# flanglet/kanzi

Measured on AMD Instinct MI355X. Metric: encode+decode MB/s, 4 MiB-block synthetic stream, BWT+RANK+ZRLT & ANS0 (level-5 core chain), bit-exact .knz, higher is better.
Workload: dtype u8; 1 GPU; configs[2]: BWT+RANK+ZRLT & ANS0, 2048 x 4194304 B blocks per GPU per step (64 distinct synthetic blocks per GPU, SURVEY 8d generator standing in for silesia.tar, tiled), blocks round-robin over ranks; block_size=4194304, parallelism=blocks%1, round_trip_ok=True

## Files before the change

kanzi_amd/csrc/kz_api.hip:

```cpp
#include <dirent.h>
#include "kz_device.h"
#include "kz_internal.h"
#include <stdlib.h>
#include <algorithm>
#include <atomic>
#include <memory>
#include <thread>
#include <chrono>
#include <sched.h>

typedef uint32_t u32;
typedef uint8_t u8;
typedef unsigned long long u64;

extern "C" int32_t kz_abi_version(void) { return KZ_ABI_VERSION; }

extern "C" kz_ctx* kz_ctx_create(int32_t deviceId) {
  int ndev = 0;
  if (hipGetDeviceCount(&ndev) != hipSuccess || ndev <= 0) return nullptr;
  if (deviceId < 0 || deviceId >= ndev) return nullptr;
  if (hipSetDevice(deviceId) != hipSuccess) return nullptr;
  kz_ctx* ctx = new kz_ctx();
  ctx->device = deviceId;
  { int cus = 0; if (hipDeviceGetAttribute(&cus, hipDeviceAttributeMultiprocessorCount, deviceId) == hipSuccess && cus > 0) ctx->numCUs = cus; }
  if (hipStreamCreateWithFlags(&ctx->stream, hipStreamNonBlocking) != hipSuccess) { delete ctx; return nullptr; }
  if (hipHostMalloc((void**)&ctx->hpin, 1 << 20, hipHostMallocDefault) != hipSuccess) { hipStreamDestroy(ctx->stream); delete ctx; return nullptr; }
  ctx->hpinInts = (1 << 20) / 4;
  kz_switches_read(ctx->sw);
  {
    const int hw = (int)std::thread::hardware_concurrency();
    ctx->blockingWaits = ctx->sw.blockingWaits >= 0 ? ctx->sw.blockingWaits : ((hw > 0 && kz_usable_cpus() < hw) ? 1 : 0);
  }
  return ctx;
}
void kz_switches_read(kz_switches& s) {
  s = kz_switches();
  auto num = [](const char* name, int unset) { const char* e = getenv(name); return e ? atoi(e) : unset; };
  auto flag = [](const char* name) { return getenv(name) != nullptr ? 1 : 0; };
  auto digit = [](const char* name, int lo, int hi, int unset) { const char* e = getenv(name); return (e && e[0] >= '0' + lo && e[0] <= '0' + hi) ? e[0] - '0' : unset; };
  { const char* e = getenv("KZ_BLOCKING_WAITS"); s.blockingWaits = e ? (atoi(e) ? 1 : 0) : -1; }
  s.textGpu = digit("KZ_TEXT_GPU", 0, 3, -1);
  s.textGpuMin = num("KZ_TEXT_GPU_MIN", 512);
  s.textFwdGpu = digit("KZ_TEXT_FWD_GPU", 0, 1, -1);
  s.textFwdGpuMin = num("KZ_TEXT_FWD_GPU_MIN", 256);
  s.utfGpu = digit("KZ_UTF_GPU", 0, 0, 1);
  s.utfFwdGpu = digit("KZ_UTF_FWD_GPU", 0, 1, -1);
  s.textGpuTrace = flag("KZ_TEXT_GPU_TRACE");
  s.fuseMinBlocks = num("KZ_FUSE_MIN_BLOCKS", 32);
  s.overlapClasses = num("KZ_OVERLAP_CLASSES", 3);
  { const char* e = getenv("KZ_WIDE_QUEUES"); s.wideQueues = e ? (atoi(e) ? 1 : 0) : -1; }
  s.noSFirst = flag("KZ_NO_SFIRST");
  s.traceSched = flag("KZ_TRACE_SCHED");
  s.tracePipe = flag("KZ_TRACE_PIPE");
  s.hostChunk = num("KZ_HOST_CHUNK", 0);
  { const int v = num("KZ_HOST_CHUNK_DEC", 512); s.hostChunkDec = v < 8 ? 8 : v; }
  { const char* e = getenv("KZ_HOST_INV_STAGED"); s.hostInvStaged = e ? atoi(e) : -1; }
  s.streamChunk = num("KZ_STREAM_CHUNK", 0);
  s.streamSerial = flag("KZ_STREAM_SERIAL");
  s.bwtTrie = num("KZ_BWT_TRIE", -1); s.bwtTrieWin = num("KZ_BWT_TRIEWIN", -1); s.bwtBuckets = num("KZ_BWT_BUCKETS", -1);
  s.bwtDmax = num("KZ_BWT_DMAX", -1); s.bwtRetire = num("KZ_BWT_RETIRE", -1); s.bwtLazyRank = num("KZ_BWT_LAZYRANK", -1);
  s.bwtTrace = flag("KZ_BWT_TRACE");
  s.bwtTestTrieOverflow = digit("KZ_BWT_TEST_TRIE_OVERFLOW", 0, 9, -1);
  { const char* f = getenv("KZ_FPAQ_FORCE"); s.fpaqForce = f ? ((f[0] == 'w' || f[0] == 'W' || f[0] == '1') ? 1 : ((f[0] == 'l' || f[0] == 'L' || f[0] == '2') ? 2 : 0)) : 0; }
  s.sbrtForm = num("KZ_SBRT_FORM", -1);
}
extern "C" void kz_ctx_reload_switches(kz_ctx* ctx) {
  if (!ctx) return;
  kz_switches_read(ctx->sw);
  if (ctx->sw.blockingWaits >= 0) ctx->blockingWaits = ctx->sw.blockingWaits;
}
extern "C" void kz_ctx_destroy(kz_ctx* ctx) {
  if (!ctx) return;
  if (ctx->worker.joinable()) {
    { std::lock_guard<std::mutex> g(ctx->qmu); ctx->stopWorker = true; }
    ctx->qcv.notify_all();
    ctx->worker.join();
  }
  hipSetDevice(ctx->device);
  if (ctx->arena) hipFree(ctx->arena);
  for (int i = 0; i < 5; i++) { if (ctx->side[i]) hipStreamDestroy(ctx->side[i]); if (ctx->evJoin[i]) hipEventDestroy(ctx->evJoin[i]); }
  if (ctx->hpin) hipHostFree(ctx->hpin);
  for (int i = 0; i < 2; i++) {
    if (ctx->pinIn[i].p) hipHostFree(ctx->pinIn[i].p);
    if (ctx->pinOut[i].p) hipHostFree(ctx->pinOut[i].p);
    if (ctx->hsIn[i].p) hipHostFree(ctx->hsIn[i].p);
    if (ctx->hsOut[i].p) hipHostFree(ctx->hsOut[i].p);
    if (ctx->tfOut[i].p) hipHostFree(ctx->tfOut[i].p);
    if (ctx->hiAux[i].p) hipFree(ctx->hiAux[i].p);
    if (ctx->hiStream[i]) hipStreamDestroy(ctx->hiStream[i]);
    if (ctx->devIn[i].p) hipFree(ctx->devIn[i].p);
    if (ctx->devOut[i].p) hipFree(ctx->devOut[i].p);
  }
  if (ctx->tfIn.p) hipHostFree(ctx->tfIn.p);
  if (ctx->tfCopy) hipStreamDestroy(ctx->tfCopy);
  if (ctx->evBlock) hipEventDestroy(ctx->evBlock);
  if (ctx->copyUp) hipStreamDestroy(ctx->copyUp);
  if (ctx->copyDown) hipStreamDestroy(ctx->copyDown);
  if (ctx->stream) hipStreamDestroy(ctx->stream);
  delete ctx;
}
extern "C" int32_t kz_ctx_set_checksum(kz_ctx* ctx, int32_t bits) {
  if (!ctx || (bits != 0 && bits != 32 && bits != 64)) return -KZ_ERR_INVALID_PARAM;
  ctx->checksum = bits == 32 ? 1 : (bits == 64 ? 2 : 0);
  return 0;
}
extern "C" int32_t kz_ctx_set_skip_blocks(kz_ctx* ctx, int32_t on) {
  if (!ctx) return -KZ_ERR_INVALID_PARAM;
  ctx->skipBlocks = on ? 1 : 0;
  return 0;
}
extern "C" int32_t kz_ctx_set_data_type(kz_ctx* ctx, int32_t dataType) {
  if (!ctx || dataType < KZ_DT_UNDEFINED || dataType > KZ_DT_UTF8) return -KZ_ERR_INVALID_PARAM;
  ctx->dataType = dataType;
  return 0;
}
extern "C" int32_t kz_ctx_set_block_size(kz_ctx* ctx, int32_t blockSize) {
  if (!ctx || blockSize < 1024 || blockSize > (1 << 30) || (blockSize & 15)) return -KZ_ERR_BLOCK_SIZE;
  ctx->blockSize = blockSize;
  ctx->blockSizeSet = true;
  return 0;
}
extern "C" int32_t kz_ctx_set_entropy(kz_ctx* ctx, uint32_t entropyType) {
  if (!ctx || entropyType >= 9 || entropyType == 3) return -KZ_ERR_INVALID_CODEC;
  ctx->entropy = (int)entropyType;
  return 0;
}
extern "C" int32_t kz_ctx_reset(kz_ctx* ctx) {
  if (!ctx) return -KZ_ERR_INVALID_PARAM;
  ctx->checksum = 0; ctx->skipBlocks = 0; ctx->dataType = KZ_DT_UNDEFINED;
  ctx->blockSize = 4 * 1024 * 1024; ctx->blockSizeSet = false; ctx->entropy = KZ_E_NONE;
  return 0;
}
extern "C" int32_t kz_ctx_get_data_type(kz_ctx* ctx) { return ctx ? ctx->dataType : -KZ_ERR_INVALID_PARAM; }
extern "C" int32_t kz_pin_to_device_numa(int32_t deviceId) {
  char bdf[64] = {0};
  if (hipDeviceGetPCIBusId(bdf, (int)sizeof(bdf), deviceId) != hipSuccess) return -KZ_ERR_DEVICE;
  for (char* p = bdf; *p; p++) if (*p >= 'A' && *p <= 'F') *p = (char)(*p - 'A' + 'a');
  char path[160];
  snprintf(path, sizeof(path), "/sys/bus/pci/devices/%s/local_cpulist", bdf);
  FILE* f = fopen(path, "r");
  if (!f) return 0;
  char line[4096] = {0};
  const bool got = fgets(line, sizeof(line), f) != nullptr;
  fclose(f);
  if (!got) return 0;
  cpu_set_t set;
  CPU_ZERO(&set);
  int count = 0;
  for (char* p = line; *p;) {
    char* e = nullptr;
    const long a = strtol(p, &e, 10);
    if (e == p) break;
    long b = a;
    p = e;
    if (*p == '-') { b = strtol(p + 1, &e, 10); p = e; }
    for (long c = a; c <= b && c < CPU_SETSIZE; c++) { CPU_SET((int)c, &set); count++; }
    if (*p == ',') p++;
  }
  if (count == 0) return 0;
  int pinned = 0;
  if (DIR* dir = opendir("/proc/self/task")) {
    while (struct dirent* de = readdir(dir)) {
      const long tid = strtol(de->d_name, nullptr, 10);
      if (tid > 0 && sched_setaffinity((pid_t)tid, sizeof(set), &set) == 0) pinned++;
    }
    closedir(dir);
  }
  if (pinned == 0 && sched_setaffinity(0, sizeof(set), &set) != 0) return 0;
  return count;
}
extern "C" const char* kz_last_error(kz_ctx* ctx) { return ctx ? ctx->err : "null context"; }
extern "C" void* kz_ctx_stream(kz_ctx* ctx) { return ctx ? (void*)ctx->stream : nullptr; }

int kz_hpin_reserve(kz_ctx* ctx, size_t ints) {
  if (ints <= ctx->hpinInts) return 0;
  KZ_HIP(kz_stream_sync(ctx, ctx->stream));
  if (ctx->hpin) { hipHostFree(ctx->hpin); ctx->hpin = nullptr; ctx->hpinInts = 0; }
  ints = kz_align(ints + (ints >> 2), 1 << 16);
  KZ_HIP(hipHostMalloc((void**)&ctx->hpin, ints * 4, hipHostMallocDefault));
  ctx->hpinInts = ints;
  return 0;
}

#define KZ_HOST_STAGE_THREADS 128
int kz_arena_reserve(kz_ctx* ctx, size_t total) {
  ctx->arenaTop = 0;
  if (total <= ctx->arenaCap) return 0;
  if (ctx->arena) { hipStreamSynchronize(ctx->stream); hipFree(ctx->arena); ctx->arena = nullptr; ctx->arenaCap = 0; }
  total = kz_align(total + (total >> 3), 1 << 20);
  KZ_HIP(hipMalloc((void**)&ctx->arena, total));
  ctx->arenaCap = total;
  return 0;
}
void* kz_arena_alloc(kz_ctx* ctx, size_t bytes) {
  size_t top = kz_align(ctx->arenaTop, 256);
  if (top + bytes > ctx->arenaCap) return nullptr;
  ctx->arenaTop = top + bytes;
  return ctx->arena + top;
}

extern "C" void kz_set_timing(kz_ctx* ctx, int32_t enable) { ctx->timing = enable != 0; }
extern "C" int32_t kz_get_stage_count(kz_ctx*) { return KZ_MAX_STAGES; }
extern "C" float kz_get_stage_ms(kz_ctx* ctx, int32_t s) { return (s >= 0 && s < KZ_MAX_STAGES) ? ctx->stageMs[s] : 0.f; }
extern "C" int64_t kz_get_stage_alg_bytes(kz_ctx* ctx, int32_t s) { return (s >= 0 && s < KZ_MAX_STAGES) ? ctx->stageAlgBytes[s] : 0; }
extern "C" void kz_reset_timing(kz_ctx* ctx) { for (int i = 0; i < KZ_MAX_STAGES; i++) { ctx->stageMs[i] = 0; ctx->stageAlgBytes[i] = 0; } }

hipEvent_t kz_ev(kz_ctx* ctx) {
  if (!ctx->evPool.empty()) { hipEvent_t e = ctx->evPool.back(); ctx->evPool.pop_back(); return e; }
  hipEvent_t e; hipEventCreate(&e); return e;
}
void kz_ktimer_flush(kz_ctx* ctx) {
  for (auto& p : ctx->pending) {
    float ms = 0;
    if (hipEventElapsedTime(&ms, p.e0, p.e1) == hipSuccess) { ctx->kMs[p.id] += ms; ctx->kLaunches[p.id]++; if (ms > ctx->kMaxMs[p.id]) ctx->kMaxMs[p.id] = ms; }
    ctx->evPool.push_back(p.e0); ctx->evPool.push_back(p.e1);
  }
  ctx->pending.clear();
}
extern "C" void kz_set_kernel_timing(kz_ctx* ctx, int32_t enable) { ctx->ktiming = enable != 0; }
extern "C" int32_t kz_get_kernel_count(void) { return KID_COUNT; }
extern "C" const char* kz_get_kernel_name(int32_t id) { static const char* n[] = KZ_KERNEL_NAMES; return (id >= 0 && id < KID_COUNT) ? n[id] : ""; }
extern "C" double kz_get_kernel_ms(kz_ctx* ctx, int32_t id) { return (id >= 0 && id < KID_COUNT) ? ctx->kMs[id] : 0.0; }
extern "C" double kz_get_kernel_max_ms(kz_ctx* ctx, int32_t id) { return (id >= 0 && id < KID_COUNT) ? ctx->kMaxMs[id] : 0.0; }
extern "C" int64_t kz_get_kernel_launches(kz_ctx* ctx, int32_t id) { return (id >= 0 && id < KID_COUNT) ? ctx->kLaunches[id] : 0; }
extern "C" void kz_reset_kernel_timing(kz_ctx* ctx) { for (int i = 0; i < KID_COUNT; i++) { ctx->kMs[i] = 0; ctx->kMaxMs[i] = 0; ctx->kLaunches[i] = 0; } }

void kz_stage_begin(kz_ctx* ctx, hipEvent_t* e0) {
  *e0 = nullptr;
  if (!ctx->timing) return;
  hipEventCreate(e0);
  hipEventRecord(*e0, ctx->stream);
}
void kz_stage_end(kz_ctx* ctx, hipEvent_t e0, int stageId, int64_t algBytes) {
  if (!ctx->timing || !e0) return;
  hipEvent_t e1; hipEventCreate(&e1);
  hipEventRecord(e1, ctx->stream);
  hipEventSynchronize(e1);
  float ms = 0; hipEventElapsedTime(&ms, e0, e1);
  ctx->stageMs[stageId] += ms; ctx->stageAlgBytes[stageId] += algBytes;
  hipEventDestroy(e0); hipEventDestroy(e1);
}

extern "C" int32_t kz_transform_max_encoded_len(uint32_t type, int32_t n) {
  switch (type) {
    case KZ_T_BWT: return n + 33;
    case KZ_T_SRT: return n + 1024;
    case KZ_T_LZ: case KZ_T_LZX: return ((n <= 1024) ? n + 16 : n + (n / 64)) + 2;
    case KZ_T_LZP: return (n <= 1024) ? n + 16 : n + (n / 64);
    case KZ_T_EXE: return (n <= 256) ? n + 32 : n + n / 8;
    case KZ_T_MM: return n + std::max(64, n >> 4);
    case KZ_T_PACK: case KZ_T_DNA: return n + 1024;
    case KZ_T_UTF: return n + 8192;
    case KZ_T_RLT: return (n <= 512) ? n + 32 : n;
    default: return n;
  }
}
extern "C" uint64_t kz_transform_type(const int32_t* types, int32_t nb) {
  uint64_t t = 0;
  for (int i = 0; i < 8; i++) t = (t << 6) | (uint64_t)((i < nb) ? (types[i] & 0x3F) : 0);
  return t;
}
static int split_types(uint64_t tt, int* types) {
  int nbtr = 0;
  for (int i = 0; i < 8; i++) if (((tt >> (42 - 6 * i)) & 0x3F) != KZ_T_NONE) nbtr++;
  if (nbtr == 0) nbtr = 1;
  int k = 0;
  for (int i = 0; i < nbtr; i++) { int t = (int)((tt >> (42 - 6 * i)) & 0x3F); if (t != KZ_T_NONE || i == 0) types[k++] = t; }
  return k;
}
static bool transform_supported(int t) { return t == KZ_T_NONE || t == KZ_T_TEXT || t == KZ_T_UTF || t == KZ_T_BWT || t == KZ_T_RANK || t == KZ_T_MTFT || t == KZ_T_ZRLT || t == KZ_T_RLT || t == KZ_T_SRT || t == KZ_T_LZ || t == KZ_T_LZX || t == KZ_T_LZP || t == KZ_T_EXE || t == KZ_T_MM || t == KZ_T_PACK || t == KZ_T_DNA; }
static bool entropy_supported(int e) { return e == KZ_E_NONE || e == KZ_E_ANS0 || e == KZ_E_ANS1 || e == KZ_E_HUFFMAN || e == KZ_E_FPAQ || e == KZ_E_RANGE; }
static bool text_codec1(int e) { return !(e == KZ_E_NONE || e == KZ_E_ANS0 || e == KZ_E_HUFFMAN || e == KZ_E_RANGE); }
int64_t kz_ans1_max_stream_bytes(int n) { return (int64_t)kz_align((size_t)n + (size_t)(n >> 3) + 1024 + 102400 * ((size_t)n / (1 << 22) + 1), 256); }
static int seq_max_len(const int* types, int nb, int n) {
  int req = n;
  for (int i = 0; i < nb; i++) req = std::max(req, kz_transform_max_encoded_len((uint32_t)types[i], req));
  return req;
}
extern "C" int64_t kz_max_block_stream_bytes(int32_t n) { return (int64_t)kz_align((size_t)n + (size_t)(n >> 3) + 1024, 256); }

__global__ void k_mask_len(const int32_t* __restrict__ len, const int32_t* __restrict__ mask, int32_t* __restrict__ out, int B) {
  const int b = blockIdx.x * blockDim.x + threadIdx.x;
  if (b < B) out[b] = mask[b] ? len[b] : 0;
}
__global__ void k_passthrough(const u8* __restrict__ src, u8* __restrict__ dst, int64_t stride, const int32_t* __restrict__ lenOld,
                              int32_t* __restrict__ lenNew, const int32_t* __restrict__ mask, const int32_t* __restrict__ flag,
                              int32_t* __restrict__ applied, const int32_t* __restrict__ part) {
  const int b = blockIdx.y;
  if (part && !part[b]) {
    if (blockIdx.x == 0 && threadIdx.x == 0) { applied[b] = 0; lenNew[b] = lenOld[b]; }
    return;
  }
  const bool ran = mask[b] != 0 && flag[b] > 0;
  if (blockIdx.x == 0 && threadIdx.x == 0) { applied[b] = ran ? 1 : ((mask[b] != 0 && flag[b] < 0) ? -1 : 0); if (!ran) lenNew[b] = lenOld[b]; }
  if (ran) return;
  const int n = lenOld[b];
  const u8* s = src + (int64_t)b * stride;
  u8* d = dst + (int64_t)b * stride;
  for (int i = (blockIdx.x * blockDim.x + threadIdx.x) * 16; i < n; i += gridDim.x * blockDim.x * 16) {
    if (i + 16 <= n) *(uint4*)(d + i) = *(const uint4*)(s + i);
    else for (int k = i; k < n; k++) d[k] = s[k];
  }
}
__global__ void k_copy_bytes(const u8* __restrict__ src, int64_t sstride, u8* __restrict__ dst, int64_t dstride,
                             const int32_t* __restrict__ len, const int32_t* __restrict__ dstOff, const int32_t* __restrict__ cond) {
  const int b = blockIdx.y;
  if (cond && !cond[b]) return;
  const int n = len[b];
  const u8* s = src + (int64_t)b * sstride;
  u8* d = dst + (int64_t)b * dstride + (dstOff ? dstOff[b] : 0);
  const int t = blockIdx.x * blockDim.x + threadIdx.x, nt = gridDim.x * blockDim.x;
  if (((((uintptr_t)s) | ((uintptr_t)d)) & 15) == 0) {
    const int n16 = n >> 4;
    for (int i = t; i < n16; i += nt) ((uint4*)d)[i] = ((const uint4*)s)[i];
    for (int i = (n16 << 4) + t; i < n; i += nt) d[i] = s[i];
  } else {
    for (int i = t; i < n; i += nt) d[i] = s[i];
  }
}

__device__ __forceinline__ u32 kz_mix32(u32 c, u32 h, u32 v) {
  c ^= h * ~v;
  c = (c << 13) | (c >> 19);
  return c * 5u + 0x52DCE729u;
}
__device__ __forceinline__ u8 kz_block_cksum(u32 mode, u32 hsf, u32 postLen, u64 written) {
  const u32 HASH = 0x1E35A7BDu;
  u32 c = HASH * 0x01030507u;
  c = kz_mix32(c, HASH, mode);
  c = kz_mix32(c, HASH, hsf);
  c = kz_mix32(c, HASH, postLen);
  c = kz_mix32(c, HASH, (u32)(written >> 32));
  c = kz_mix32(c, HASH, (u32)written);
  c = (c >> 23) ^ (c >> 3);
  return (u8)c;
}

struct FrameEnc {
  int32_t* postLen;
  int32_t* skipFlags;
  int32_t* hdrBytes;
  int32_t* isCopy;
  int32_t* fallback;
  int64_t* bits;
  u64* hash;
  int chk;
  int nbFunctions;
};

__global__ void k_frame_prepare(FrameEnc F, int B) {
  const int b = blockIdx.x * blockDim.x + threadIdx.x;
  if (b >= B) return;
  const int postLen = F.postLen[b];
  const int dataSize = (postLen < 256) ? 1 : (kz_ilog2((u32)postLen) >> 3) + 1;
  const bool two = !F.isCopy[b] && F.nbFunctions > 4;
  F.hdrBytes[b] = 1 + (two ? 1 : 0) + dataSize + 1 + (F.chk == 1 ? 4 : (F.chk == 2 ? 8 : 0));
}
__global__ void k_frame_decide(FrameEnc F, int B) {
  const int b = blockIdx.x * blockDim.x + threadIdx.x;
  if (b >= B) return;
  const int64_t written = 8LL * F.hdrBytes[b] + F.bits[b];
  const int64_t entropyBytes = (written + 7) >> 3;
  F.fallback[b] = (!F.isCopy[b] && (int64_t)F.postLen[b] < entropyBytes) ? 1 : 0;
// ... 1683 lines not shown
```

kanzi_amd/csrc/kz_bwt_fwd.hip:

```cpp
#include "kz_device.h"
#include "kz_internal.h"
#include <stdlib.h>
#include <algorithm>

#define RS_ITEMS 16
#define RS_TILE (KZ_WG * RS_ITEMS)
#define BW_LIVE 0x80000000u
#define RSORT_TILE 16384
#define RSORT_ITEMS (RSORT_TILE / KZ_WG)

typedef unsigned long long u64;
typedef uint32_t u32;
typedef uint8_t u8;
typedef u64 __attribute__((aligned(1))) bw_u64_unaligned;

struct BwtArrays {
  u64* key[2]; u32* val[2];
  u32* rank; u32* sa;
  u32* tileHist;
  u32* digitBase;
  u32* bucketCnt;
  int32_t* d_w;
  int32_t* d_big;
  u32* tileA;
// ... 118 lines not shown
  const int b = bw_row_block(A, blockIdx.y);
  const int w0 = MSD ? 0 : A.d_w[b];
  const int m = A.d_m[b] - w0;
  const int tile = blockIdx.x;
  if ((int64_t)tile * RSORT_TILE >= m) return;
  __shared__ CNT cnt[RSC_WAVES][BINS];
  __shared__ u32 gdelta[BINS];
  __shared__ u32 scan[32];
  __shared__ u64 stage[RSORT_TILE];
  for (int i = threadIdx.x; i < RSC_WAVES * BINS; i += RSC_WG) (&cnt[0][0])[i] = 0;
  __syncthreads();
  const int64_t off = (int64_t)b * A.NS + w0;
  const int wave = threadIdx.x >> 6;
  const int lane = kz_lane();
  const int tbase = tile * RSORT_TILE;
  const int base = tbase + wave * (64 * RSC_ITEMS);
  const int tcount = min(RSORT_TILE, m - tbase);
  const uint64_t lt = kz_lanemask_lt();
  u64 k[RSC_ITEMS]; u32 v[RSC_ITEMS]; u32 dr[RSC_ITEMS];
#pragma unroll
  for (int r = 0; r < RSC_ITEMS; r++) {
    const int idx = base + r * 64 + lane;
    const bool valid = idx < m;
    if (TEXT) {
      k[r] = valid ? bw_text_key(X.src + (int64_t)b * X.stride, idx, m, X.K) : 0;
      v[r] = (u32)idx;
    } else {
      k[r] = valid ? keyIn[off + idx] : 0;
      v[r] = valid ? valIn[off + idx] : 0;
    }
  }
#pragma unroll
  for (int r = 0; r < RSC_ITEMS; r++) {
    const int idx = base + r * 64 + lane;
    const bool valid = idx < m;
    const u32 d = (u32)((k[r] >> shift) & (BINS - 1));
    const uint64_t vm = kz_ballot(valid);
    const u32 d0 = (u32)__builtin_amdgcn_readfirstlane((int)d);
    const bool uni = (vm != 0) && (kz_ballot(valid && d == d0) == vm);
    const uint64_t peers = uni ? (valid ? vm : 0ULL) : bw_match<NBITS>(d, valid);
    u32 pre = 0;
    if (valid) pre = cnt[wave][d];
    const u32 rnk = pre + (u32)__popcll(peers & lt);
    if (valid && (peers >> lane) == 1ULL) cnt[wave][d] = (CNT)(pre + (u32)__popcll(peers));
    dr[r] = d | (rnk << 16);
  }
  __syncthreads();
  {
    u32 tot = 0;
    u32 c[RSC_WAVES];
    const int d = threadIdx.x & (BINS - 1);
#pragma unroll
    for (int w = 0; w < RSC_WAVES; w++) { c[w] = cnt[w][d]; tot += c[w]; }
    u32 total;
    const u32 ts = kz_wg_excl_sum(threadIdx.x < BINS ? tot : 0u, scan, &total);
    if (threadIdx.x < BINS) {
      gdelta[d] = A.digitBase[b * MSD_BINS + d] + A.tileHist[(int64_t)b * A.HS + (int64_t)tile * BINS + d] - ts;
      u32 run = ts;
#pragma unroll
      for (int w = 0; w < RSC_WAVES; w++) { cnt[w][d] = (CNT)run; run += c[w]; }
    }
  }
  __syncthreads();
#pragma unroll
  for (int r = 0; r < RSC_ITEMS; r++) {
    const int idx = base + r * 64 + lane;
    if (idx < m) { const u32 slot = cnt[wave][dr[r] & 0xFFFF] + (dr[r] >> 16); dr[r] = slot; stage[slot] = k[r]; }
  }
  __syncthreads();
  u32 gp[RSC_ITEMS];
#pragma unroll
  for (int r = 0; r < RSC_ITEMS; r++) {
    const int slot = r * RSC_WG + threadIdx.x;
    if (slot < tcount) {
      const u64 kk = stage[slot];
      gp[r] = gdelta[(u32)((kk >> shift) & (BINS - 1))] + (u32)slot;
      keyOut[off + gp[r]] = kk;
    }
  }
  __syncthreads();
  u32* stageV = (u32*)stage;
#pragma unroll
  for (int r = 0; r < RSC_ITEMS; r++) {
    const int idx = base + r * 64 + lane;
    if (idx < m) stageV[dr[r]] = v[r];
  }
  __syncthreads();
#pragma unroll
  for (int r = 0; r < RSC_ITEMS; r++) {
    const int slot = r * RSC_WG + threadIdx.x;
    if (slot < tcount) valOut[off + gp[r]] = stageV[slot];
  }
}
__global__ __launch_bounds__(RSC_WG) void k_radix_scatter(const u64* __restrict__ keyIn, const u32* __restrict__ valIn,
                                                           u64* __restrict__ keyOut, u32* __restrict__ valOut,
                                                           BwtArrays A, int shift) { radix_scatter_body<256, 8, false, u32, false>(keyIn, valIn, keyOut, valOut, A, shift, TextSrc{nullptr, 0, 0}); }
__global__ __launch_bounds__(RSC_WG) void k_radix_scatter0(u64* __restrict__ keyOut, u32* __restrict__ valOut, BwtArrays A, TextSrc X) {
  radix_scatter_body<256, 8, false, u32, true>(nullptr, nullptr, keyOut, valOut, A, 0, X);
}
__global__ __launch_bounds__(RSC_WG) void k_msd_scatter(const u64* __restrict__ keyIn, const u32* __restrict__ valIn,
                                                         u64* __restrict__ keyOut, u32* __restrict__ valOut,
                                                         BwtArrays A, int shift) {
  const int b = bw_row_block(A, blockIdx.y);
  const int m = A.d_m[b];
  const int tile = blockIdx.x;
  if ((int64_t)tile * RSORT_TILE >= m) return;
  __shared__ u32 cnt[MSD_BINS];
  __shared__ u32 gdelta[MSD_BINS];
  __shared__ u32 scan[32];
  __shared__ u64 stage[RSORT_TILE];
  cnt[threadIdx.x] = 0;
  __syncthreads();
  const int64_t off = (int64_t)b * A.NS;
  const int lane = kz_lane();
  const int tbase = tile * RSORT_TILE;
  const int tcount = min(RSORT_TILE, m - tbase);
  const uint64_t lt = kz_lanemask_lt();
  u64 k[RSC_ITEMS]; u32 v[RSC_ITEMS]; u32 dr[RSC_ITEMS];
#pragma unroll
  for (int r = 0; r < RSC_ITEMS; r++) {
    const int idx = tbase + r * RSC_WG + threadIdx.x;
    const bool valid = idx < m;
    k[r] = valid ? keyIn[off + idx] : 0;
    v[r] = valid ? valIn[off + idx] : 0;
  }
#pragma unroll
  for (int r = 0; r < RSC_ITEMS; r++) {
    const int idx = tbase + r * RSC_WG + threadIdx.x;
    const bool valid = idx < m;
    const u32 d = (u32)(k[r] >> shift) & (MSD_BINS - 1);
    const uint64_t vm = kz_ballot(valid);
    const u32 d0 = (u32)__builtin_amdgcn_readfirstlane((int)d);
    u32 pos = 0;
    if (vm != 0 && kz_ballot(valid && d == d0) == vm) {
      u32 basePos = 0;
      if (lane == (int)__builtin_ctzll(vm)) basePos = atomicAdd(&cnt[d0], (u32)__popcll(vm));
      basePos = (u32)__shfl((int)basePos, (int)__builtin_ctzll(vm), 64);
      pos = basePos + (u32)__popcll(vm & lt);
    } else if (valid) pos = atomicAdd(&cnt[d], 1u);
    dr[r] = pos;
  }
  __syncthreads();
  {
    const u32 tot = cnt[threadIdx.x];
    u32 total;
    const u32 ts = kz_wg_excl_sum(tot, scan, &total);
    gdelta[threadIdx.x] = A.digitBase[b * MSD_BINS + threadIdx.x] + A.tileHist[(int64_t)b * A.HS + (int64_t)tile * MSD_BINS + threadIdx.x] - ts;
    cnt[threadIdx.x] = ts;
  }
  __syncthreads();
#pragma unroll
  for (int r = 0; r < RSC_ITEMS; r++) {
    const int idx = tbase + r * RSC_WG + threadIdx.x;
    if (idx < m) { const u32 slot = cnt[(u32)(k[r] >> shift) & (MSD_BINS - 1)] + dr[r]; dr[r] = slot; stage[slot] = k[r]; }
  }
  __syncthreads();
  u32 gp[RSC_ITEMS];
#pragma unroll
  for (int r = 0; r < RSC_ITEMS; r++) {
    const int slot = r * RSC_WG + threadIdx.x;
    if (slot < tcount) {
      const u64 kk = stage[slot];
      gp[r] = gdelta[(u32)(kk >> shift) & (MSD_BINS - 1)] + (u32)slot;
      keyOut[off + gp[r]] = kk;
    }
  }
  __syncthreads();
  u32* stageV = (u32*)stage;
#pragma unroll
  for (int r = 0; r < RSC_ITEMS; r++) {
    const int idx = tbase + r * RSC_WG + threadIdx.x;
    if (idx < m) stageV[dr[r]] = v[r];
  }
  __syncthreads();
#pragma unroll
  for (int r = 0; r < RSC_ITEMS; r++) {
    const int slot = r * RSC_WG + threadIdx.x;
    if (slot < tcount) valOut[off + gp[r]] = stageV[slot];
  }
}

__device__ __forceinline__ u32 bw_group(u64 k, int gshift) { return gshift >= 64 ? 0u : (u32)(k >> gshift); }

__device__ __forceinline__ void bw_row_flags(const u64* __restrict__ key, int base, int m, int gshift, int lane,
                                             u64 (&k)[RS_ITEMS], uint64_t (&hb)[RS_ITEMS], uint64_t (&sb)[RS_ITEMS]) {
  u64 prevRowLast = (base > 0 && base <= m) ? key[base - 1] : 0;
#pragma unroll
  for (int r = 0; r < RS_ITEMS; r++) {
    const int c = base + r * 64 + lane;
    k[r] = (c < m) ? key[c] : 0;
    u64 prev = __shfl_up(k[r], 1, 64);
    if (lane == 0) prev = prevRowLast;
    const bool valid = c < m;
    const bool head = valid && (c == 0 || k[r] != prev);
    const bool seg = head && (c == 0 || bw_group(k[r], gshift) != bw_group(prev, gshift));
    hb[r] = kz_ballot(head);
    sb[r] = kz_ballot(seg);
    prevRowLast = __shfl(k[r], 63, 64);
  }
}

__global__ __launch_bounds__(KZ_WG) void k_seg_reduce(const u64* __restrict__ keyS, BwtArrays A, int gshift) {
  const int b = bw_row_block(A, blockIdx.y);
  const int w0 = A.d_w[b];
  const int m = A.d_m[b] - w0;
  const int tile = blockIdx.x;
  if ((int64_t)tile * RS_TILE >= m) return;
  __shared__ u32 wS[4], wH[4];
  const u64* key = keyS + (int64_t)b * A.NS + w0;
  const int wave = threadIdx.x >> 6, lane = kz_lane();
  const int base = tile * RS_TILE + wave * (64 * RS_ITEMS);
  u64 k[RS_ITEMS]; uint64_t hb[RS_ITEMS], sb[RS_ITEMS];
  bw_row_flags(key, base, m, gshift, lane, k, hb, sb);
  u32 ms = 0, mh = 0;
#pragma unroll
  for (int r = 0; r < RS_ITEMS; r++) {
    if (hb[r]) mh = (u32)(base + r * 64 + 63 - (int)__builtin_clzll(hb[r])) + 1;
    if (sb[r]) ms = (u32)(base + r * 64 + 63 - (int)__builtin_clzll(sb[r])) + 1;
  }
  if (lane == 0) { wS[wave] = ms; wH[wave] = mh; }
  __syncthreads();
  if (threadIdx.x == 0) {
    A.tileA[(int64_t)b * A.T + tile] = max(max(wS[0], wS[1]), max(wS[2], wS[3]));
    A.tileB[(int64_t)b * A.T + tile] = max(max(wH[0], wH[1]), max(wH[2], wH[3]));
  }
}
__global__ void k_seg_scan(BwtArrays A) {
  const int b = bw_row_block(A, blockIdx.x);
  const int m = A.d_m[b] - A.d_w[b];
  const int tiles = (m + RS_TILE - 1) / RS_TILE;
  u32* ta = A.tileA + (int64_t)b * A.T;
  u32* tb = A.tileB + (int64_t)b * A.T;
  u32 ca = 0, cb = 0;
  for (int base = 0; base < tiles; base += 64) {
    const int i = base + threadIdx.x;
    const u32 va = (i < tiles) ? ta[i] : 0, vb = (i < tiles) ? tb[i] : 0;
    const u32 ia = kz_wave_incl_max(va), ib = kz_wave_incl_max(vb);
    u32 ea = __shfl_up(ia, 1, 64), eb = __shfl_up(ib, 1, 64);
    if (threadIdx.x == 0) { ea = 0; eb = 0; }
    ea = ea > ca ? ea : ca; eb = eb > cb ? eb : cb;
    if (i < tiles) { ta[i] = ea; tb[i] = eb; }
    const u32 la = __shfl(ia, 63, 64), lb = __shfl(ib, 63, 64);
    ca = ca > la ? ca : la; cb = cb > lb ? cb : lb;
  }
}
__global__ __launch_bounds__(KZ_WG) void k_seg_apply(const u64* __restrict__ keyS, const u32* __restrict__ valS, BwtArrays A, int gshift) {
  const int b = bw_row_block(A, blockIdx.y);
  const int w0 = A.d_w[b];
  const int m = A.d_m[b] - w0;
  const int tile = blockIdx.x;
  if ((int64_t)tile * RS_TILE >= m) return;
  __shared__ u32 wS[4], wH[4];
  const int64_t off = (int64_t)b * A.NS;
  const u64* key = keyS + off + w0;
  const int wave = threadIdx.x >> 6, lane = kz_lane();
  const int base = tile * RS_TILE + wave * (64 * RS_ITEMS);
  u64 k[RS_ITEMS]; uint64_t hb[RS_ITEMS], sb[RS_ITEMS];
  bw_row_flags(key, base, m, gshift, lane, k, hb, sb);
  u32 ms = 0, mh = 0;
#pragma unroll
  for (int r = 0; r < RS_ITEMS; r++) {
    if (hb[r]) mh = (u32)(base + r * 64 + 63 - (int)__builtin_clzll(hb[r])) + 1;
    if (sb[r]) ms = (u32)(base + r * 64 + 63 - (int)__builtin_clzll(sb[r])) + 1;
  }
  if (lane == 0) { wS[wave] = ms; wH[wave] = mh; }
  __syncthreads();
  u32 carS = A.tileA[(int64_t)b * A.T + tile], carH = A.tileB[(int64_t)b * A.T + tile];
  for (int w = 0; w < wave; w++) { carS = max(carS, wS[w]); carH = max(carH, wH[w]); }
  u32* rank = A.rank + off;
  u32* sa = A.sa + off;
  const u32* val = valS + off + w0;
  const uint64_t le = kz_lanemask_lt() | (1ULL << lane);
  const u64 afterLast = (base + 64 * RS_ITEMS < m) ? key[base + 64 * RS_ITEMS] : 0;
#pragma unroll
  for (int r = 0; r < RS_ITEMS; r++) {
    const int rowBase = base + r * 64;
    const int c = rowBase + lane;
    const uint64_t hbl = hb[r] & le, sbl = sb[r] & le;
    const u32 hh = hbl ? (u32)(rowBase + 63 - (int)__builtin_clzll(hbl)) : carH - 1;
    const u32 ss = sbl ? (u32)(rowBase + 63 - (int)__builtin_clzll(sbl)) : carS - 1;
    u64 nextk = __shfl_down(k[r], 1, 64);
    const u64 nextRowFirst = (r + 1 < RS_ITEMS) ? __shfl(k[(r + 1 < RS_ITEMS) ? r + 1 : r], 0, 64) : afterLast;
    if (lane == 63) nextk = nextRowFirst;
    if (c < m) {
      const u32 g = bw_group(k[r], gshift);
      const bool headC = hh == (u32)c;
      const bool headN = (c + 1 >= m) || (nextk != k[r]);
      const u32 sv = val[c];
      const bool live = !(headC && headN);
      if (!(live && hh == ss && gshift < 64)) rank[sv] = (g + (hh - ss)) | (live ? BW_LIVE : 0u);
      if (!live) sa[g + ((u32)c - ss)] = sv;
    }
    if (hb[r]) carH = (u32)(rowBase + 63 - (int)__builtin_clzll(hb[r])) + 1;
    if (sb[r]) carS = (u32)(rowBase + 63 - (int)__builtin_clzll(sb[r])) + 1;
  }
}

#define BK_DBITS 9
#define BK_DBINS (1 << BK_DBITS)
#define BK_SMALL 1024
#define BK_SORT 0x40000000u
static_assert(RSC_WG == MSD_BINS, "k_msd_scatter geometry");

template <int WAVES, int ROWS>
__device__ __forceinline__ void bucket_body(const u64* __restrict__ keyS, const u32* __restrict__ valS, const BwtArrays& A, int bitsR, int bitsG) {
  const int b = bw_row_block(A, blockIdx.y);
  const u32 d = blockIdx.x;
  const u32 bc0 = A.bucketCnt[b * MSD_BINS + d];
  if ((bc0 & (BK_SORT | BK_BIG)) != BK_SORT) return;
  const u32 bc = bc0 & ~BK_SORT;
  const int cnt = (int)bc;
  const int wave = threadIdx.x >> 6, lane = kz_lane();
  __shared__ u64 buf[WAVES * ROWS * 64];
  __shared__ uint16_t cw[WAVES][BK_DBINS];
  __shared__ u32 wsum[BK_DBINS / 64];
  __shared__ u32 wS[WAVES], wH[WAVES];
  __shared__ int skip[8];
  const int64_t off = (int64_t)b * A.NS;
  const u32 bo = A.digitBase[b * MSD_BINS + d];
  const int rows = (cnt + 63) >> 6;
  const int R = (rows + WAVES - 1) / WAVES;
  const int base = wave * R * 64;
  const uint64_t lt = kz_lanemask_lt();
  const u64 kbase = (u64)d << (bitsR + BK_BITS);
  u64 k[ROWS]; u32 dr[ROWS];
#pragma unroll
  for (int r = 0; r < ROWS; r++) {
    const int idx = base + r * 64 + lane;
    k[r] = ~0ULL;
    if (r < R && idx < cnt) k[r] = ((keyS[off + bo + idx] - kbase) << bitsG) | (u64)valS[off + bo + idx];
  }
  {
    if (threadIdx.x < 8) skip[threadIdx.x] = 0;
    const int keyBits = bitsR + BK_BITS;
    const int passes = (keyBits + BK_DBITS - 1) / BK_DBITS;
    for (int p = 0; p < passes; p++) {
      const int shift = bitsG + BK_DBITS * p;
      for (int i = threadIdx.x; i < WAVES * BK_DBINS / 2; i += WAVES * 64) ((u32*)&cw[0][0])[i] = 0;
      __syncthreads();
#pragma unroll
      for (int r = 0; r < ROWS; r++) {
        if (r < R) {
          const int idx = base + r * 64 + lane;
          const bool valid = idx < cnt;
          const u32 dg = (u32)(k[r] >> shift) & (BK_DBINS - 1);
          const uint64_t vm = kz_ballot(valid);
          if (vm == 0) continue;
          const u32 d0 = (u32)__builtin_amdgcn_readfirstlane((int)dg);
          const bool uni = kz_ballot(valid && dg == d0) == vm;
          const uint64_t peers = uni ? (valid ? vm : 0ULL) : bw_match<BK_DBITS>(dg, valid);
          u32 pre = 0;
          if (valid) pre = cw[wave][dg];
          const u32 rnk = pre + (u32)__popcll(peers & lt);
          if (valid && (peers >> lane) == 1ULL) cw[wave][dg] = (uint16_t)(pre + (u32)__popcll(peers));
          dr[r] = dg | (rnk << 16);
        }
      }
      __syncthreads();
      constexpr int DPT = (BK_DBINS + WAVES * 64 - 1) / (WAVES * 64);
      u32 c[DPT][WAVES]; u32 tot[DPT]; u32 mine = 0;
#pragma unroll
      for (int q = 0; q < DPT; q++) {
        const int dg = threadIdx.x * DPT + q;
        tot[q] = 0;
        if (dg < BK_DBINS) {
#pragma unroll
          for (int w = 0; w < WAVES; w++) { c[q][w] = cw[w][dg]; tot[q] += c[q][w]; }
          if (tot[q] == (u32)cnt) skip[p] = 1;
        }
        mine += tot[q];
      }
      const u32 inc = kz_wave_incl_sum(mine);
      if (lane == 63 && wave < BK_DBINS / 64) wsum[wave] = inc;
      __syncthreads();
      if (skip[p]) continue;
      {
        u32 run = inc - mine;
        for (int w = 0; w < wave && w < BK_DBINS / 64; w++) run += wsum[w];
#pragma unroll
        for (int q = 0; q < DPT; q++) {
          const int dg = threadIdx.x * DPT + q;
          if (dg < BK_DBINS) {
#pragma unroll
            for (int w = 0; w < WAVES; w++) { cw[w][dg] = (uint16_t)run; run += c[q][w]; }
          }
        }
      }
      __syncthreads();
#pragma unroll
      for (int r = 0; r < ROWS; r++) {
        if (r < R) {
          const int idx = base + r * 64 + lane;
          if (idx < cnt) buf[cw[wave][dr[r] & 0xFFFF] + (dr[r] >> 16)] = k[r];
        }
      }
      __syncthreads();
#pragma unroll
      for (int r = 0; r < ROWS; r++) {
        if (r < R) {
          const int idx = base + r * 64 + lane;
          if (idx < cnt) k[r] = buf[idx];
        }
      }
      __syncthreads();
    }
#pragma unroll
    for (int r = 0; r < ROWS; r++) {
      if (r < R) {
        const int idx = base + r * 64 + lane;
        if (idx < cnt) buf[idx] = k[r];
      }
    }
    __syncthreads();
  }
  uint64_t hb[ROWS], sb[ROWS];
  u32 ms = 0, mh = 0;
  const int gsh = bitsG + bitsR;
#pragma unroll
  for (int r = 0; r < ROWS; r++) {
    hb[r] = 0; sb[r] = 0;
    if (r < R) {
      const int idx = base + r * 64 + lane;
      const bool valid = idx < cnt;
      const u64 prev = (valid && idx > 0) ? buf[idx - 1] : 0;
      const bool head = valid && (idx == 0 || (k[r] >> bitsG) != (prev >> bitsG));
      const bool seg = head && (idx == 0 || (k[r] >> gsh) != (prev >> gsh));
      hb[r] = kz_ballot(head);
      sb[r] = kz_ballot(seg);
      if (hb[r]) mh = (u32)(base + r * 64 + 63 - (int)__builtin_clzll(hb[r])) + 1;
      if (sb[r]) ms = (u32)(base + r * 64 + 63 - (int)__builtin_clzll(sb[r])) + 1;
    }
  }
  u32 carS = 0, carH = 0;
  {
    if (lane == 0) { wS[wave] = ms; wH[wave] = mh; }
    __syncthreads();
    for (int w = 0; w < wave; w++) { carS = max(carS, wS[w]); carH = max(carH, wH[w]); }
  }
  u32* rank = A.rank + off;
  u32* sa = A.sa + off;
  const uint64_t le = lt | (1ULL << lane);
  const u64 vmask = (1ULL << bitsG) - 1ULL;
  const u32 gbase = d << BK_BITS;
#pragma unroll
  for (int r = 0; r < ROWS; r++) {
    if (r < R) {
      const int rowBase = base + r * 64;
      const int idx = rowBase + lane;
      const uint64_t hbl = hb[r] & le, sbl = sb[r] & le;
      const u32 hh = hbl ? (u32)(rowBase + 63 - (int)__builtin_clzll(hbl)) : carH - 1;
      const u32 ss = sbl ? (u32)(rowBase + 63 - (int)__builtin_clzll(sbl)) : carS - 1;
      if (idx < cnt) {
        const u64 nextk = (idx + 1 < cnt) ? buf[idx + 1] : 0;
        const bool headC = hh == (u32)idx;
        const bool headN = (idx + 1 >= cnt) || ((nextk >> bitsG) != (k[r] >> bitsG));
        const bool live = !(headC && headN);
        const u32 g = gbase + (u32)(k[r] >> gsh);
        const u32 sv = (u32)(k[r] & vmask);
        if (!(live && hh == ss)) rank[sv] = (g + (hh - ss)) | (live ? BW_LIVE : 0u);
        if (!live) sa[g + ((u32)idx - ss)] = sv;
      }
      if (hb[r]) carH = (u32)(rowBase + 63 - (int)__builtin_clzll(hb[r])) + 1;
      if (sb[r]) carS = (u32)(rowBase + 63 - (int)__builtin_clzll(sb[r])) + 1;
    }
  }
}
__global__ __launch_bounds__(1024, 8) void k_bucket_sort(const u64* __restrict__ keyS, const u32* __restrict__ valS, BwtArrays A, int bitsR, int bitsG) {
  bucket_body<16, BK_CAP / 1024>(keyS, valS, A, bitsR, bitsG);
}

#define BK_GMAX 256
#define BK_SLOTS (1 << BK_BITS)
template <int WAVES, int ROWS, int LO, int HI, typename CNT>
__device__ __forceinline__ void bucket_count_body(const u64* __restrict__ keyS, const u32* __restrict__ valS, const BwtArrays& A, int bitsR, int bitsG, u32 gmax) {
  const int b = bw_row_block(A, blockIdx.y);
  const u32 d = blockIdx.x;
  const u32 bc = A.bucketCnt[b * MSD_BINS + d];
  if (bc <= (u32)LO || bc > (u32)HI) return;
  const int cnt = (int)bc;
  const int wave = threadIdx.x >> 6, lane = kz_lane();
  const bool tiny = LO == 0 && cnt <= 64;
  if (tiny && wave != 0) return;
  const int64_t off = (int64_t)b * A.NS;
  const u32 bo = A.digitBase[b * MSD_BINS + d];
  u32* rank = A.rank + off;
  u32* sa = A.sa + off;
  const u32 gbase = d << BK_BITS;
  const u32 rmask = (1u << bitsR) - 1u;
  constexpr int WG = WAVES * 64;
  if (tiny) {
    const bool valid = lane < cnt;
    const u64 key = valid ? keyS[off + bo + lane] : ~0ULL;
    const u32 sv = valid ? valS[off + bo + lane] : 0u;
    const u32 gv = (u32)(key >> bitsR), rv = (u32)key & rmask;
    u32 rk = 0, eq = 0;
    for (int j = 0; j < cnt; j++) {
      const u32 gj = (u32)__builtin_amdgcn_readlane((int)gv, j), rj = (u32)__builtin_amdgcn_readlane((int)rv, j);
      if (gj == gv) { rk += (rj < rv) ? 1u : 0u; eq += (rj == rv) ? 1u : 0u; }
    }
    if (valid) {
      const bool live = eq > 1;
      if (!(live && rk == 0)) rank[sv] = (gv + rk) | (live ? BW_LIVE : 0u);
      if (!live) sa[gv + rk] = sv;
    }
    return;
  }
  __shared__ u64 buf[WAVES * ROWS * 64];
  __shared__ CNT start[BK_SLOTS];
  __shared__ u32 wsum[WAVES];
  __shared__ u32 gmaxS;
  for (int i = threadIdx.x; i < BK_SLOTS; i += WG) start[i] = 0;
  if (threadIdx.x == 0) gmaxS = 0;
  __syncthreads();
  const u64 kbase = (u64)d << (bitsR + BK_BITS);
  u64 k[ROWS]; u32 pos[ROWS];
#pragma unroll
  for (int r = 0; r < ROWS; r++) {
    const int idx = r * WG + threadIdx.x;
    k[r] = 0; pos[r] = 0;
    if (idx < cnt) {
      k[r] = ((keyS[off + bo + idx] - kbase) << bitsG) | (u64)valS[off + bo + idx];
      pos[r] = (u32)atomicAdd(&start[(u32)(k[r] >> (bitsG + bitsR))], (CNT)1);
    }
  }
  __syncthreads();
  {
    constexpr int SPT = BK_SLOTS / WG;
    u32 c[SPT]; u32 mine = 0, gm = 0;
#pragma unroll
    for (int q = 0; q < SPT; q++) { c[q] = start[threadIdx.x * SPT + q]; mine += c[q]; gm = max(gm, c[q]); }
    const u32 inc = kz_wave_incl_sum(mine);
    if (lane == 63) wsum[wave] = inc;
    if (gm > gmax) atomicMax(&gmaxS, gm);
    __syncthreads();
    u32 run = inc - mine;
    for (int w = 0; w < wave; w++) run += wsum[w];
#pragma unroll
    for (int q = 0; q < SPT; q++) { start[threadIdx.x * SPT + q] = (CNT)run; run += c[q]; }
  }
  __syncthreads();
  if (gmaxS > gmax) {
    if (threadIdx.x == 0) A.bucketCnt[b * MSD_BINS + d] = bc | BK_SORT;
    return;
  }
#pragma unroll
  for (int r = 0; r < ROWS; r++) {
    const int idx = r * WG + threadIdx.x;
    if (idx < cnt) buf[(u32)start[(u32)(k[r] >> (bitsG + bitsR))] + pos[r]] = k[r];
  }
  __syncthreads();
  const u64 vmask = (1ULL << bitsG) - 1ULL;
#pragma unroll
  for (int r = 0; r < ROWS; r++) {
    const int idx = r * WG + threadIdx.x;
    if (idx < cnt) {
      const u64 e = buf[idx];
      const u32 grel = (u32)(e >> (bitsG + bitsR));
      const u32 rv = (u32)(e >> bitsG) & rmask;
      const int gs = (int)start[grel];
      const int ge = (grel + 1 < (u32)BK_SLOTS) ? (int)start[grel + 1] : cnt;
      u32 rk = 0, eq = 0;
      int j = gs;
      for (; j + 4 <= ge; j += 4) {
        const u64 e0 = buf[j], e1 = buf[j + 1], e2 = buf[j + 2], e3 = buf[j + 3];
        const u32 r0 = (u32)(e0 >> bitsG) & rmask, r1 = (u32)(e1 >> bitsG) & rmask, r2_ = (u32)(e2 >> bitsG) & rmask, r3 = (u32)(e3 >> bitsG) & rmask;
        rk += (r0 < rv) + (r1 < rv) + (r2_ < rv) + (r3 < rv);
        eq += (r0 == rv) + (r1 == rv) + (r2_ == rv) + (r3 == rv);
      }
      for (; j < ge; j++) {
        const u32 rj = (u32)(buf[j] >> bitsG) & rmask;
        rk += (rj < rv) ? 1u : 0u; eq += (rj == rv) ? 1u : 0u;
      }
      const u32 sv = (u32)(e & vmask);
      const u32 g = gbase + grel;
      const bool live = eq > 1;
      if (!(live && rk == 0)) rank[sv] = (g + rk) | (live ? BW_LIVE : 0u);
      if (!live) sa[g + rk] = sv;
    }
  }
}
__global__ __launch_bounds__(256) void k_bucket_count_s(const u64* __restrict__ keyS, const u32* __restrict__ valS, BwtArrays A, int bitsR, int bitsG, u32 gmax) {
  bucket_count_body<4, BK_SMALL / 256, 0, BK_SMALL, u32>(keyS, valS, A, bitsR, bitsG, gmax);
}
__global__ __launch_bounds__(1024) void k_bucket_count(const u64* __restrict__ keyS, const u32* __restrict__ valS, BwtArrays A, int bitsR, int bitsG, u32 gmax) {
  bucket_count_body<16, BK_CAP / 1024, BK_SMALL, BK_CAP, u32>(keyS, valS, A, bitsR, bitsG, gmax);
}

#define TR_META 32
__global__ __launch_bounds__(KZ_WG) void k_live_emit(u64* __restrict__ keyN, u32* __restrict__ valN, BwtArrays A, int h, int bitsR, int first, const int32_t* __restrict__ lazyMeta) {
  const int b = bw_row_block(A, blockIdx.y);
  const int n = A.d_n[b];
  const int tile = blockIdx.x;
  if ((int64_t)tile * RS_TILE >= n) return;
  if (lazyMeta && lazyMeta[(int64_t)b * TR_META] == 256 && lazyMeta[(int64_t)b * TR_META + 18] == 0 && lazyMeta[(int64_t)b * TR_META + 20] == 0) {
    if (threadIdx.x == 0) A.tileLive[(int64_t)b * A.T + tile] = 0;
    return;
  }
  if (!first && A.tileLive[(int64_t)b * A.T + tile] == 0) return;
  __shared__ u32 rowCnt[RS_ITEMS * 4 + 1];
  __shared__ u32 tileBase;
  const int64_t off = (int64_t)b * A.NS;
  const u32* rank = A.rank + off;
  const int wave = threadIdx.x >> 6, lane = kz_lane();
  const int base = tile * RS_TILE + wave * (64 * RS_ITEMS);
  u32 rk[RS_ITEMS];
  uint64_t bal[RS_ITEMS];
#pragma unroll
  for (int r = 0; r < RS_ITEMS; r++) {
    const int s = base + r * 64 + lane;
    rk[r] = (s < n) ? rank[s] : 0u;
    bal[r] = kz_ballot((rk[r] & BW_LIVE) != 0);
    if (lane == 0) rowCnt[wave * RS_ITEMS + r] = (u32)__popcll(bal[r]);
  }
  __syncthreads();
  if (threadIdx.x < 64) {
    const u32 v = rowCnt[threadIdx.x];
    const u32 inc = kz_wave_incl_sum(v);
    rowCnt[threadIdx.x] = inc - v;
    if (threadIdx.x == 63) {
      const u32 tot = inc;
      A.tileLive[(int64_t)b * A.T + tile] = tot;
      tileBase = tot ? (u32)atomicAdd(&A.d_m2[b], (int32_t)tot) : 0u;
    }
  }
  __syncthreads();
  const u32 tbase = tileBase;
  const uint64_t lt = kz_lanemask_lt();
  const u32 hcap = (u32)min(h, n);
#pragma unroll
  for (int r = 0; r < RS_ITEMS; r++) {
    if (rk[r] & BW_LIVE) {
      const int s = base + r * 64 + lane;
      const int64_t j = (int64_t)s + h;
      const u64 r2 = (j < n) ? (u64)(rank[j] & ~BW_LIVE) + (u64)hcap + 1ULL : (u64)(n - s);
      const u32 pos = tbase + rowCnt[wave * RS_ITEMS + r] + (u32)__popcll(bal[r] & lt);
      keyN[off + pos] = ((u64)(rk[r] & ~BW_LIVE) << bitsR) | r2;
      valN[off + pos] = (u32)s;
    }
  }
}

#if defined(__HIP_DEVICE_COMPILE__) && !defined(__gfx950__)
#error "the trie rounds are sized for gfx950's 160 KiB of LDS per workgroup (k_tr_hist16 128 KiB, k_tr_scatter / k_trk_scatter 152 KiB, the bucket sorts 77 KiB)"
#endif
#define TR_CAP 7680u
#define TR_MERGE (TR_CAP / 2)
#define TR_K_SMALL 1u
#define TR_K_EXP 2u
#define TR_K_TERM 3u
#define TR_UNCHANGED (1u << 29)
#define TR_NODECHUNK 128
struct TrieArrays {
  u32* cnt;
  u32* info;
  u32* nodeStart;
  u32* bStart;
  u32* bCount;
  u32* bFill;
  u32* bAux;
  u32* bG;
  u32* nodePfx;
  u32* nodeGS;
  int32_t* meta;
  int32_t* err;
  int MN, MB;
};

__device__ __forceinline__ u32 tr_byte(const u8* __restrict__ s, int i, int n) { return i < n ? (u32)s[i] : 0u; }

__global__ __launch_bounds__(1024) void k_tr_hist16(const u8* __restrict__ srcAll, int64_t stride, BwtArrays A, TrieArrays T) {
  const int b = blockIdx.y;
  const int n = A.d_n[b];
  const u32 half = blockIdx.x;
  __shared__ u32 hist[32768];
  for (int i = threadIdx.x; i < 32768; i += 1024) hist[i] = 0;
  __syncthreads();
  const u8* s = srcAll + (int64_t)b * stride;
  const int lane = kz_lane();
  for (int base = 0; base < n; base += 1024 * 16) {
    const int p = base + threadIdx.x * 16;
    uint4 q = make_uint4(0, 0, 0, 0);
    if (p < n) q = *(const uint4*)(s + p);
    u32 nxt = (u32)__shfl_down((int)(q.x & 0xFFu), 1, 64);
    if (lane == 63) nxt = (p + 16 < n) ? (u32)s[p + 16] : 0u;
    const u32 w[5] = {q.x, q.y, q.z, q.w, nxt};
    u32 runKey = 0xFFFFFFFFu, runCnt = 0;
#pragma unroll
    for (int j = 0; j < 16; j++) {
      const int i = p + j;
      const u32 c0 = (w[j >> 2] >> ((j & 3) * 8)) & 0xFFu;
      const u32 c1r = (w[(j + 1) >> 2] >> (((j + 1) & 3) * 8)) & 0xFFu;
      const u32 c1 = (i + 1 < n) ? c1r : 0u;
      const u32 key = (c0 << 8) | c1;
      const bool mine = i < n && (key >> 15) == half;
      if (mine && key == runKey) runCnt++;
      else {
        if (runCnt) atomicAdd(&hist[runKey & 32767u], runCnt);
        runKey = mine ? key : 0xFFFFFFFFu; runCnt = mine ? 1u : 0u;
      }
    }
    if (runCnt) atomicAdd(&hist[runKey & 32767u], runCnt);
  }
  __syncthreads();
  u32* out = T.cnt + (int64_t)b * T.MN * 256 + half * 32768;
  for (int i = threadIdx.x; i < 32768; i += 1024) out[i] = hist[i];
}

__global__ __launch_bounds__(256) void k_tr_assign(BwtArrays A, TrieArrays T, int L, int Dmax, int keys) {
  const int b = bw_row_block(A, blockIdx.x);
  int32_t* meta = T.meta + (int64_t)b * TR_META;
  __shared__ u32 sNodes, sBuckets, sErr;
  __shared__ u32 scan[32];
  const int lo = (L == 1) ? 0 : meta[2 + L], hi = (L == 1) ? 256 : meta[10 + L];
  if (threadIdx.x == 0) { sNodes = (L == 1) ? 256u : (u32)meta[0]; sBuckets = (L == 1) ? 0u : (u32)meta[1]; sErr = 0; }
  __syncthreads();
  const u32 firstNew = sNodes;
  u32* cnt = T.cnt + (int64_t)b * T.MN * 256;
  u32* info = T.info + (int64_t)b * T.MN * 256;
  u32* nodeStart = T.nodeStart + (int64_t)b * T.MN;
  u32* bStart = T.bStart + (int64_t)b * T.MB;
  u32* bCount = T.bCount + (int64_t)b * T.MB;
  u32* bAux = T.bAux + (int64_t)b * T.MB;
  u32* bG = T.bG + (int64_t)b * T.MB;
  u32* nodePfx = T.nodePfx + (int64_t)b * T.MN;
  u32* nodeGS = T.nodeGS + (int64_t)b * T.MN;
  const u32 skipTag = (u32)L << 16;
  for (int base = lo; base < hi; base += 256) {
    const int node = base + threadIdx.x;
    const bool valid = node < hi;
    u32 start = 0;
    if (L == 1) {
      u32 tot = 0;
      for (int c = 0; c < 256; c += 4) {
        const uint4 v = *(const uint4*)(cnt + (int64_t)node * 256 + c);
        tot += v.x + v.y + v.z + v.w;
      }
      u32 total;
      start = kz_wg_excl_sum(tot, scan, &total);
      nodeStart[node] = start;
      if (keys) nodePfx[node] = (u32)node;
    } else if (valid) start = nodeStart[node];
    if (!valid) continue;
    u32 run = start, curCnt = 0;
    int curB = -1;
    const u32 pfxN = keys ? nodePfx[node] : 0u;
    const u32 gsN = (keys && L >= 3) ? nodeGS[node] : 0u;
    const u32 auxSmall = !keys ? 0u : (L >= 3 ? pfxN - gsN : pfxN);
    for (int c4 = 0; c4 < 256; c4 += 4) {
      const uint4 v4 = *(const uint4*)(cnt + (int64_t)node * 256 + c4);
      const u32 cc4[4] = {v4.x, v4.y, v4.z, v4.w};
#pragma unroll
      for (int j = 0; j < 4; j++) {
        const u32 cc = cc4[j];
        if (cc == 0) continue;
        const u32 s0 = run;
        run += cc;
        u32 e;
        const u32 cbyte = (u32)(c4 + j);
        if (cc > TR_CAP) {
          if (curB >= 0) { bCount[curB] = curCnt | skipTag; curB = -1; }
          if (L + 1 < Dmax) {
            const u32 M = atomicAdd(&sNodes, 1u);
            if (M < (u32)T.MN) {
              nodeStart[M] = s0; e = (TR_K_EXP << 30) | M;
              uint4* z = (uint4*)(cnt + (int64_t)M * 256);
              for (int q = 0; q < 64; q++) z[q] = make_uint4(0, 0, 0, 0);
              if (keys) { nodePfx[M] = (L < 3) ? ((pfxN << 8) | cbyte) : pfxN; nodeGS[M] = (L + 1 == 3) ? s0 : gsN; }
            } else { sErr = 1; e = (TR_K_TERM << 30) | s0; }
          } else if (keys) {
            const u32 head = pfxN + (s0 - gsN);
            e = (TR_K_TERM << 30) | (s0 == gsN ? TR_UNCHANGED : 0u) | (head & 0xFFFFFFu);
          } else e = (TR_K_TERM << 30) | s0;
        } else if (cc > TR_MERGE) {
          if (curB >= 0) { bCount[curB] = curCnt | skipTag; curB = -1; }
          const u32 id = atomicAdd(&sBuckets, 1u);
          if (id < (u32)T.MB) { bStart[id] = s0; bCount[id] = cc | skipTag; bAux[id] = (keys && L >= 3) ? auxSmall + s0 : auxSmall; bG[id] = pfxN; } else sErr = 1;
          e = (TR_K_SMALL << 30) | ((u32)L << 16) | (id & 0xFFFFu);
        } else {
          if (curB >= 0 && curCnt + cc <= TR_CAP) curCnt += cc;
          else {
            if (curB >= 0) bCount[curB] = curCnt | skipTag;
            const u32 id = atomicAdd(&sBuckets, 1u);
            if (id < (u32)T.MB) { bStart[id] = s0; curB = (int)id; bAux[id] = (keys && L >= 3) ? auxSmall + s0 : auxSmall; bG[id] = pfxN; } else { sErr = 1; curB = -1; }
            curCnt = cc;
          }
          e = (TR_K_SMALL << 30) | ((u32)L << 16) | ((u32)curB & 0xFFFFu);
        }
        info[(int64_t)node * 256 + c4 + j] = e;
      }
    }
    if (curB >= 0) bCount[curB] = curCnt | skipTag;
  }
  __syncthreads();
  if (threadIdx.x == 0) {
    meta[0] = (int32_t)min(sNodes, (u32)T.MN); meta[1] = (int32_t)min(sBuckets, (u32)T.MB);
    meta[2 + L + 1] = (int32_t)firstNew; meta[10 + L + 1] = (int32_t)min(sNodes, (u32)T.MN);
    if (sErr) { meta[18] = 1; atomicOr(T.err, 1); }
  }
}

#define TRC_U 4
__global__ __launch_bounds__(1024) void k_tr_count(const u8* __restrict__ srcAll, int64_t stride, u32* __restrict__ stateAll, BwtArrays A, TrieArrays T, int L) {
  const int b = blockIdx.y;
  const int32_t* meta = T.meta + (int64_t)b * TR_META;
  const int lo = meta[2 + L], hi = meta[10 + L];
  if (hi <= lo) return;
  const int n = A.d_n[b];
  __shared__ u32 lds[TR_NODECHUNK * 256];
  const u8* s = srcAll + (int64_t)b * stride;
  u32* state = stateAll + (int64_t)b * A.NS;
  const u32* info = T.info + (int64_t)b * T.MN * 256;
  u32* cnt = T.cnt + (int64_t)b * T.MN * 256;
  const int P = gridDim.x;
  const int per = (((n + P - 1) / P) + 1023) & ~1023;
  const int pbeg = blockIdx.x * per, pend = min(n, pbeg + per);
  for (int chunk = 0; lo + chunk * TR_NODECHUNK < hi; chunk++) {
    for (int i = threadIdx.x; i < TR_NODECHUNK * 256; i += 1024) lds[i] = 0;
    __syncthreads();
    const int nlo = lo + chunk * TR_NODECHUNK;
    for (int i0 = pbeg; i0 < pend; i0 += TRC_U * 4096) {
      uint4 st4[TRC_U]; u64 win[TRC_U]; bool any[TRC_U];
#pragma unroll
      for (int u = 0; u < TRC_U; u++) {
        const int i = i0 + u * 4096 + threadIdx.x * 4;
        any[u] = i < pend;
        st4[u] = make_uint4(0xC0000000u, 0xC0000000u, 0xC0000000u, 0xC0000000u);
        win[u] = 0;
        if (any[u]) {
          if (!(L == 2 && chunk == 0)) st4[u] = *(const uint4*)(state + i);
          const int at = i + L - 2;
          u64 k = __builtin_bswap64(*(const bw_u64_unaligned*)(s + at));
          const int rem = n - at;
          if (rem < 8) k = rem <= 0 ? 0ULL : (k & (~0ULL << (8 * (8 - rem))));
          win[u] = k;
        }
      }
      u32 stqA[TRC_U][4]; u32 eA[TRC_U][4]; bool lookA[TRC_U][4];
#pragma unroll
      for (int u = 0; u < TRC_U; u++) {
        const int i = i0 + u * 4096 + threadIdx.x * 4;
        stqA[u][0] = st4[u].x; stqA[u][1] = st4[u].y; stqA[u][2] = st4[u].z; stqA[u][3] = st4[u].w;
#pragma unroll
        for (int q = 0; q < 4; q++) {
          if (L == 2 && chunk == 0) stqA[u][q] = (any[u] && i + q < pend) ? ((1u << 16) | (u32)((win[u] >> (56 - 8 * q)) & 0xFFu)) : 0xC0000000u;
          lookA[u][q] = any[u] && (i + q < pend) && (stqA[u][q] >> 30) == 0 && ((stqA[u][q] >> 16) & 7u) != (u32)L;
          eA[u][q] = 0;
          if (lookA[u][q]) eA[u][q] = info[(stqA[u][q] & 0xFFFFu) * 256 + (u32)((win[u] >> (48 - 8 * q)) & 0xFFu)];
        }
      }
#pragma unroll
      for (int u = 0; u < TRC_U; u++) {
        if (!any[u]) continue;
        const int i = i0 + u * 4096 + threadIdx.x * 4;
        u32 (&stq)[4] = stqA[u];
        u32 (&e)[4] = eA[u]; bool (&look)[4] = lookA[u];
        bool changed = false;
        u32 runT = 0xFFFFFFFFu, runC = 0;
#pragma unroll
        for (int q = 0; q < 4; q++) {
          u32 tgt = 0xFFFFFFFFu;
          if ((i + q < pend) && (stq[q] >> 30) == 0) {
            if (look[q]) {
              stq[q] = ((e[q] >> 30) == TR_K_EXP) ? ((e[q] & 0xFFFFu) | ((u32)L << 16)) : e[q];
              changed = true;
            }
            if ((stq[q] >> 30) == 0) {
              const int k = (int)(stq[q] & 0xFFFFu) - nlo;
              if (k >= 0 && k < TR_NODECHUNK) tgt = (u32)k * 256 + (u32)((win[u] >> (40 - 8 * q)) & 0xFFu);
            }
          }
          if (tgt == runT) runC++;
          else {
            if (runC && runT != 0xFFFFFFFFu) atomicAdd(&lds[runT], runC);
            runT = tgt; runC = 1;
          }
        }
        if (runC && runT != 0xFFFFFFFFu) atomicAdd(&lds[runT], runC);
        if (changed) *(uint4*)(state + i) = make_uint4(stq[0], stq[1], stq[2], stq[3]);
      }
    }
    __syncthreads();
    for (int j = threadIdx.x; j < TR_NODECHUNK * 256; j += 1024) {
      const u32 v = lds[j];
      if (v && nlo + (j >> 8) < hi) atomicAdd(&cnt[(int64_t)(nlo + (j >> 8)) * 256 + (j & 255)], v);
    }
    __syncthreads();
  }
}

#define TRS_TILE 8192
#define TRS_ITEMS (TRS_TILE / 1024)
#define TR_MAXB 12288
#define TRS_FASTB 2048
template <int TILE_, int MAXB_, bool FAST>
__device__ __forceinline__ void tr_scatter_body(const u8* __restrict__ srcAll, int64_t stride, const u32* __restrict__ stateAll,
                                                u64* __restrict__ elemAll, const BwtArrays& A, const TrieArrays& T, int bitsG) {
  constexpr int ITEMS_ = TILE_ / 1024;
  if ((T.meta[(int64_t)blockIdx.y * TR_META + 1] <= TRS_FASTB) != FAST) return;
  const int b = blockIdx.y;
  const int n = A.d_n[b];
  const int tile = blockIdx.x;
  const int tbase = tile * TILE_;
  if (tbase >= n) return;
  __shared__ u32 tc2[MAXB_ / 2];
  __shared__ u32 gdelta[MAXB_];
  __shared__ u64 stage[TILE_];
  __shared__ uint16_t stageB[TILE_];
  __shared__ u32 scan[32];
  const int32_t* meta = T.meta + (int64_t)b * TR_META;
  const int nB = meta[1];
  const bool hasState = meta[10 + 2] > meta[2 + 2];
  for (int i = threadIdx.x; i < (nB + 1) / 2; i += 1024) tc2[i] = 0;
  __syncthreads();
  const u8* s = srcAll + (int64_t)b * stride;
  const u32* state = stateAll + (int64_t)b * A.NS;
  const u32* info = T.info + (int64_t)b * T.MN * 256;
  u32* rank = A.rank + (int64_t)b * A.NS;
  const u64 lowMask = (1ULL << bitsG) - 1ULL;
  u64 el[ITEMS_]; u32 bp[ITEMS_];
  u32 stv[ITEMS_];
#pragma unroll
  for (int r = 0; r < ITEMS_; r++) {
    const int i = tbase + r * 1024 + threadIdx.x;
    stv[r] = 0xC0000000u;
    if (i < n) stv[r] = hasState ? state[i] : ((u32)s[i] | (1u << 16));
  }
  u32 cb[ITEMS_];
#pragma unroll
  for (int r = 0; r < ITEMS_; r++) {
    const int i = tbase + r * 1024 + threadIdx.x;
    cb[r] = 0;
    if (i < n && (stv[r] >> 30) == 0) cb[r] = tr_byte(s, i + (int)((stv[r] >> 16) & 7u), n);
  }
#pragma unroll
  for (int r = 0; r < ITEMS_; r++) {
    const int i = tbase + r * 1024 + threadIdx.x;
    if (i < n && (stv[r] >> 30) == 0) stv[r] = info[(stv[r] & 0xFFFFu) * 256 + cb[r]];
  }
  u64 kv[ITEMS_];
#pragma unroll
  for (int r = 0; r < ITEMS_; r++) {
    const int i = tbase + r * 1024 + threadIdx.x;
    kv[r] = 0;
    if (i < n && (stv[r] >> 30) != TR_K_TERM) {
      const int at = i + (int)((stv[r] >> 16) & 7u);
      u64 k = __builtin_bswap64(*(const bw_u64_unaligned*)(s + at));
      const int rem = n - at;
      if (rem < 8) k = rem <= 0 ? 0ULL : (k & (~0ULL << (8 * (8 - rem))));
      kv[r] = k;
    }
  }
#pragma unroll
  for (int r = 0; r < ITEMS_; r++) {
    const int i = tbase + r * 1024 + threadIdx.x;
    bp[r] = 0xFFFFFFFFu;
    el[r] = 0;
    if (i < n) {
      const u32 st = stv[r];
      if ((st >> 30) == TR_K_TERM) rank[i] = (st & 0xFFFFFFu) | BW_LIVE;
      else {
        const u32 bk = st & 0xFFFFu;
        el[r] = (kv[r] & ~lowMask) | (u64)(u32)i;
        const u32 old = atomicAdd(&tc2[bk >> 1], (bk & 1u) ? 65536u : 1u);
        const u32 pos = (bk & 1u) ? (old >> 16) : (old & 0xFFFFu);
        bp[r] = bk | (pos << 16);
      }
    }
  }
  __syncthreads();
  {
    const int per = 2 * ((nB + 2047) / 2048);
    const int j0 = threadIdx.x * per;
    u32 mine = 0;
    for (int j = j0; j < j0 + per && j < nB; j += 2) { const u32 w = tc2[j >> 1]; mine += (w & 0xFFFFu) + (w >> 16); }
    u32 total;
    u32 run = kz_wg_excl_sum(mine, scan, &total);
    const u32* bStart = T.bStart + (int64_t)b * T.MB;
    u32* bFill = T.bFill + (int64_t)b * T.MB;
    for (int j = j0; j < j0 + per && j < nB; j += 2) {
      const u32 w = tc2[j >> 1];
      const u32 c0 = w & 0xFFFFu, c1 = w >> 16;
      if (c0) gdelta[j] = bStart[j] + atomicAdd(&bFill[j], c0) - run;
      const u32 r1 = run + c0;
      if (c1) gdelta[j + 1] = bStart[j + 1] + atomicAdd(&bFill[j + 1], c1) - r1;
      tc2[j >> 1] = run | (r1 << 16);
      run = r1 + c1;
    }
    if (threadIdx.x == 0) scan[31] = total;
  }
  __syncthreads();
  const u32 total = scan[31];
#pragma unroll
  for (int r = 0; r < ITEMS_; r++) {
    if (bp[r] != 0xFFFFFFFFu) {
      const u32 bk = bp[r] & 0xFFFFu;
      const u32 w = tc2[bk >> 1];
      const u32 slot = ((bk & 1u) ? (w >> 16) : (w & 0xFFFFu)) + (bp[r] >> 16);
      stage[slot] = el[r]; stageB[slot] = (uint16_t)bk;
    }
  }
  __syncthreads();
  u64* elem = elemAll + (int64_t)b * A.NS;
#pragma unroll
  for (int r = 0; r < ITEMS_; r++) {
    const u32 slot = (u32)r * 1024 + threadIdx.x;
    if (slot < total) elem[gdelta[stageB[slot]] + slot] = stage[slot];
  }
}

__global__ __launch_bounds__(1024) void k_tr_scatter(const u8* __restrict__ srcAll, int64_t stride, const u32* __restrict__ stateAll,
                                                      u64* __restrict__ elemAll, BwtArrays A, TrieArrays T, int bitsG) { tr_scatter_body<TRS_TILE, TR_MAXB, false>(srcAll, stride, stateAll, elemAll, A, T, bitsG); }
__global__ __launch_bounds__(1024) void k_tr_scatter_f(const u8* __restrict__ srcAll, int64_t stride, const u32* __restrict__ stateAll,
                                                        u64* __restrict__ elemAll, BwtArrays A, TrieArrays T, int bitsG) { tr_scatter_body<TRS_TILE / 2, TRS_FASTB, true>(srcAll, stride, stateAll, elemAll, A, T, bitsG); }

__device__ __forceinline__ bool tr_lazy_candidate(const int32_t* meta) { return meta[0] == 256 && meta[18] == 0; }
#define TRQ_WAVES 16
#define TRQ_ROWS 8
template <bool KEYS>
__device__ __forceinline__ void tr_sort_body(const u64* __restrict__ elemAll, const BwtArrays& A, const TrieArrays& T, int bitsG, int lazyMode) {
  const int b = bw_row_block(A, blockIdx.y);
  const int nB = T.meta[(int64_t)b * TR_META + 1];
  const bool lazyCand = !KEYS && lazyMode != 0 && tr_lazy_candidate(T.meta + (int64_t)b * TR_META);
  if (!KEYS && lazyMode == 2 && !(lazyCand && T.meta[(int64_t)b * TR_META + 20] > 0)) return;
  const bool lazy = lazyCand && lazyMode == 1;
  u32 pstep = 0;
  if (lazy) { const int n = A.d_n[b]; const int st = n >> 3; pstep = (u32)((st * 8 != n) ? st + 1 : st); }
  u32 liveMine = 0;
  __shared__ u64 buf[TR_CAP];
  __shared__ uint16_t cw[TRQ_WAVES][BK_DBINS];
  __shared__ u32 wsum[BK_DBINS / 64];
  __shared__ u32 wH[TRQ_WAVES], wS[TRQ_WAVES];
  __shared__ u64 redO[TRQ_WAVES], redA[TRQ_WAVES];
  __shared__ int skip[8];
  const int wave = threadIdx.x >> 6, lane = kz_lane();
  const int64_t off = (int64_t)b * A.NS;
  const u64* elem = elemAll + off;
  u32* rank = A.rank + off;
  u32* sa = A.sa + off;
  const uint64_t lt = kz_lanemask_lt();
  const uint64_t le = lt | (1ULL << lane);
  const u64 vmask = (1ULL << bitsG) - 1ULL;
  for (int d = blockIdx.x; d < nB; d += gridDim.x) {
    const u32 bcs = T.bCount[(int64_t)b * T.MB + d];
    const int cnt = (int)(bcs & 0xFFFFu);
    const int skipB = (int)(bcs >> 16);
    const u32 bo = T.bStart[(int64_t)b * T.MB + d];
    const u32 aux = KEYS ? T.bAux[(int64_t)b * T.MB + d] : 0u;
    const u32 gOne = KEYS ? T.bG[(int64_t)b * T.MB + d] : 0u;
    const int rows = (cnt + 63) >> 6;
    const int R = (rows + TRQ_WAVES - 1) / TRQ_WAVES;
    const int base = wave * R * 64;
    u64 k[TRQ_ROWS]; u32 dr[TRQ_ROWS];
    u64 vo = 0, va = ~0ULL;
#pragma unroll
    for (int r = 0; r < TRQ_ROWS; r++) {
      const int idx = base + r * 64 + lane;
      k[r] = ~0ULL;
      if (r < R && idx < cnt) { k[r] = elem[bo + idx]; vo |= k[r]; va &= k[r]; }
    }
    for (int dd = 32; dd > 0; dd >>= 1) { vo |= __shfl_xor(vo, dd, 64); va &= __shfl_xor(va, dd, 64); }
    if (threadIdx.x < 8) skip[threadIdx.x] = 0;
    if (lane == 0) { redO[wave] = vo; redA[wave] = va; }
    __syncthreads();
    vo = 0; va = ~0ULL;
#pragma unroll
    for (int w = 0; w < TRQ_WAVES; w++) { vo |= redO[w]; va &= redA[w]; }
    const u64 diff = (vo ^ va) >> bitsG;
    int passes = 0, lowBit = 0;
    if (diff) {
      lowBit = (int)__builtin_ctzll(diff);
      const int hiBit = 63 - (int)__builtin_clzll(diff);
      passes = (hiBit - lowBit + BK_DBITS) / BK_DBITS;
    }
    for (int p = 0; p < passes; p++) {
      const int shift = bitsG + lowBit + BK_DBITS * p;
      for (int i = threadIdx.x; i < TRQ_WAVES * BK_DBINS / 2; i += TRQ_WAVES * 64) ((u32*)&cw[0][0])[i] = 0;
      __syncthreads();
#pragma unroll
      for (int r = 0; r < TRQ_ROWS; r++) {
        if (r < R) {
          const int idx = base + r * 64 + lane;
          const bool valid = idx < cnt;
          const u32 dg = (u32)(k[r] >> shift) & (BK_DBINS - 1);
          const uint64_t vm = kz_ballot(valid);
          if (vm == 0) continue;
          const u32 d0 = (u32)__builtin_amdgcn_readfirstlane((int)dg);
          const bool uni = kz_ballot(valid && dg == d0) == vm;
          const uint64_t peers = uni ? (valid ? vm : 0ULL) : bw_match<BK_DBITS>(dg, valid);
          u32 pre = 0;
          if (valid) pre = cw[wave][dg];
          const u32 rnk = pre + (u32)__popcll(peers & lt);
          if (valid && (peers >> lane) == 1ULL) cw[wave][dg] = (uint16_t)(pre + (u32)__popcll(peers));
          dr[r] = dg | (rnk << 16);
        }
      }
      __syncthreads();
      static_assert(BK_DBINS <= TRQ_WAVES * 64, "one digit per thread");
      u32 mine = 0;
      if (threadIdx.x < BK_DBINS) {
#pragma unroll
        for (int w = 0; w < TRQ_WAVES; w++) mine += cw[w][threadIdx.x];
        if (mine == (u32)cnt) skip[p] = 1;
      }
      const u32 inc = kz_wave_incl_sum(mine);
      if (lane == 63 && wave < BK_DBINS / 64) wsum[wave] = inc;
      __syncthreads();
      if (skip[p]) continue;
      if (threadIdx.x < BK_DBINS) {
        u32 run = inc - mine;
        for (int w = 0; w < wave; w++) run += wsum[w];
#pragma unroll
        for (int w = 0; w < TRQ_WAVES; w++) { const u32 cv = cw[w][threadIdx.x]; cw[w][threadIdx.x] = (uint16_t)run; run += cv; }
      }
      __syncthreads();
#pragma unroll
      for (int r = 0; r < TRQ_ROWS; r++) {
        if (r < R) {
          const int idx = base + r * 64 + lane;
          if (idx < cnt) buf[cw[wave][dr[r] & 0xFFFF] + (dr[r] >> 16)] = k[r];
        }
      }
      __syncthreads();
#pragma unroll
      for (int r = 0; r < TRQ_ROWS; r++) {
        if (r < R) {
          const int idx = base + r * 64 + lane;
          if (idx < cnt) k[r] = buf[idx];
        }
      }
      __syncthreads();
    }
#pragma unroll
    for (int r = 0; r < TRQ_ROWS; r++) {
      if (r < R) {
        const int idx = base + r * 64 + lane;
        if (idx < cnt) buf[idx] = k[r];
      }
    }
    __syncthreads();
    const bool segs = KEYS && skipB < 3;
    const int gsh = 64 - 8 * (3 - skipB);
    u32 mh = 0, ms = 0;
#pragma unroll
    for (int r = 0; r < TRQ_ROWS; r++) {
      if (r < R) {
        const int idx = base + r * 64 + lane;
        const bool valid = idx < cnt;
        const u64 prev = (valid && idx > 0) ? buf[idx - 1] : 0;
        const bool head = valid && (idx == 0 || (k[r] >> bitsG) != (prev >> bitsG));
        const uint64_t hbr = kz_ballot(head);
        if (hbr) mh = (u32)(base + r * 64 + 63 - (int)__builtin_clzll(hbr)) + 1;
        if (segs) {
          const uint64_t sbr = kz_ballot(head && (idx == 0 || (k[r] >> gsh) != (prev >> gsh)));
          if (sbr) ms = (u32)(base + r * 64 + 63 - (int)__builtin_clzll(sbr)) + 1;
        }
      }
    }
    if (lane == 0) { wH[wave] = mh; wS[wave] = ms; }
    __syncthreads();
    u32 carH = 0, carS = 0;
    for (int w = 0; w < wave; w++) { carH = max(carH, wH[w]); carS = max(carS, wS[w]); }
#pragma unroll
    for (int r = 0; r < TRQ_ROWS; r++) {
      if (r < R) {
        const int rowBase = base + r * 64;
        const int idx = rowBase + lane;
        const bool valid = idx < cnt;
        const u64 prev = (valid && idx > 0) ? buf[idx - 1] : 0;
        const bool head = valid && (idx == 0 || (k[r] >> bitsG) != (prev >> bitsG));
        const uint64_t hbr = kz_ballot(head);
        const uint64_t hbl = hbr & le;
        const u32 hh = hbl ? (u32)(rowBase + 63 - (int)__builtin_clzll(hbl)) : carH - 1;
        uint64_t sbr = 0;
        u32 ss = 0;
        if (segs) {
          sbr = kz_ballot(head && (idx == 0 || (k[r] >> gsh) != (prev >> gsh)));
          const uint64_t sbl = sbr & le;
          ss = sbl ? (u32)(rowBase + 63 - (int)__builtin_clzll(sbl)) : carS - 1;
        }
        if (valid) {
          const u64 nextk = (idx + 1 < cnt) ? buf[idx + 1] : 0;
          const bool headN = (idx + 1 >= cnt) || ((nextk >> bitsG) != (k[r] >> bitsG));
          const bool live = !(hh == (u32)idx && headN);
          const u32 sv = (u32)(k[r] & vmask);
          if (!KEYS) {
            if (!lazy) rank[sv] = (bo + hh) | (live ? BW_LIVE : 0u);
            else {
              const u32 q = sv / pstep;
              if (q * pstep == sv && q < 8u) rank[sv] = (bo + hh) | (live ? BW_LIVE : 0u);
              liveMine += live ? 1u : 0u;
            }
            if (!live) sa[bo + (u32)idx] = sv;
          } else {
            u32 g, headSlot, slot;
            if (segs) {
              g = (aux << (8 * (3 - skipB))) | (u32)(k[r] >> gsh);
              headSlot = g + (hh - ss); slot = g + ((u32)idx - ss);
            } else { g = gOne; headSlot = aux + hh; slot = aux + (u32)idx; }
            if (!(live && headSlot == g)) rank[sv] = headSlot | (live ? BW_LIVE : 0u);
            if (!live) sa[slot] = sv;
          }
        }
        if (hbr) carH = (u32)(rowBase + 63 - (int)__builtin_clzll(hbr)) + 1;
        if (sbr) carS = (u32)(rowBase + 63 - (int)__builtin_clzll(sbr)) + 1;
      }
    }
    __syncthreads();
  }
  if (!KEYS && lazy) {
    if (kz_ballot(liveMine != 0) != 0) {
      for (int dd = 32; dd > 0; dd >>= 1) liveMine += __shfl_xor(liveMine, dd, 64);
      if (lane == 0) atomicAdd(&T.meta[(int64_t)b * TR_META + 20], (int32_t)liveMine);
    }
  }
}
__global__ __launch_bounds__(1024, 8) void k_tr_sort(const u64* __restrict__ elemAll, BwtArrays A, TrieArrays T, int bitsG, int lazyMode) { tr_sort_body<false>(elemAll, A, T, bitsG, lazyMode); }
__global__ __launch_bounds__(1024, 8) void k_trk_sort(const u64* __restrict__ elemAll, BwtArrays A, TrieArrays T, int bitsG) { tr_sort_body<true>(elemAll, A, T, bitsG, 0); }

struct KeySrc { const u64* key; const u32* val; int bitsR; };
__device__ __forceinline__ u64 trk_k48(u64 key, int bitsR) { return ((key >> bitsR) << 24) | (key & ((1ULL << bitsR) - 1ULL)); }

__global__ __launch_bounds__(1024) void k_trk_hist16(KeySrc X, BwtArrays A, TrieArrays T) {
  const int b = bw_row_block(A, blockIdx.y);
  const int w0 = A.d_w[b];
  const int W = max(0, A.d_m[b] - w0);
  const u32 half = blockIdx.x;
  __shared__ u32 hist[32768];
  for (int i = threadIdx.x; i < 32768; i += 1024) hist[i] = 0;
  __syncthreads();
  const u64* key = X.key + (int64_t)b * A.NS + w0;
  const int lane = kz_lane();
  for (int j0 = 0; j0 < W; j0 += 1024) {
    const int j = j0 + threadIdx.x;
    u32 tgt = 0xFFFFFFFFu;
    if (j < W) {
      const u32 pair = (u32)(trk_k48(key[j], X.bitsR) >> 32);
      if ((pair >> 15) == half) tgt = pair & 32767u;
    }
    const uint64_t am = kz_ballot(tgt != 0xFFFFFFFFu);
    if (am) {
      const int l0 = (int)__builtin_ctzll(am);
      const u32 t0 = (u32)__shfl((int)tgt, l0, 64);
      const uint64_t same = kz_ballot(tgt == t0);
      if (lane == l0) atomicAdd(&hist[t0], (u32)__popcll(same));
      else if (tgt != 0xFFFFFFFFu && tgt != t0) atomicAdd(&hist[tgt], 1u);
    }
  }
  __syncthreads();
  u32* out = T.cnt + (int64_t)b * T.MN * 256 + half * 32768;
  for (int i = threadIdx.x; i < 32768; i += 1024) out[i] = hist[i];
}

__global__ __launch_bounds__(1024) void k_trk_count(KeySrc X, u32* __restrict__ stateAll, BwtArrays A, TrieArrays T, int L) {
  const int b = bw_row_block(A, blockIdx.y);
  const int32_t* meta = T.meta + (int64_t)b * TR_META;
  const int lo = meta[2 + L], hi = meta[10 + L];
  if (hi <= lo) return;
  const int w0 = A.d_w[b];
  const int W = A.d_m[b] - w0;
  __shared__ u32 lds[TR_NODECHUNK * 256];
  const u64* key = X.key + (int64_t)b * A.NS + w0;
  u32* state = stateAll + (int64_t)b * A.NS;
  const u32* info = T.info + (int64_t)b * T.MN * 256;
  u32* cnt = T.cnt + (int64_t)b * T.MN * 256;
  const int P = gridDim.x;
  const int per = (((W + P - 1) / P) + 1023) & ~1023;
  const int pbeg = blockIdx.x * per, pend = min(W, pbeg + per);
  for (int chunk = 0; lo + chunk * TR_NODECHUNK < hi; chunk++) {
    for (int i = threadIdx.x; i < TR_NODECHUNK * 256; i += 1024) lds[i] = 0;
    __syncthreads();
    const int nlo = lo + chunk * TR_NODECHUNK;
    for (int i0 = pbeg; i0 < pend; i0 += TRC_U * 4096) {
      u64 kq[TRC_U][4]; u32 stq[TRC_U][4]; bool act[TRC_U];
#pragma unroll
      for (int u = 0; u < TRC_U; u++) {
        const int i = i0 + u * 4096 + (int)threadIdx.x * 4;
        act[u] = i < pend;
#pragma unroll
        for (int q = 0; q < 4; q++) { stq[u][q] = 0xC0000000u; kq[u][q] = 0; }
        if (!act[u]) continue;
        if (!(L == 2 && chunk == 0)) {
          const uint4 sv = *(const uint4*)(state + i);
          stq[u][0] = sv.x; stq[u][1] = sv.y; stq[u][2] = sv.z; stq[u][3] = sv.w;
          if ((stq[u][0] >> 30) && (stq[u][1] >> 30) && (stq[u][2] >> 30) && (stq[u][3] >> 30)) { act[u] = false; continue; }
        }
        if (i + 4 <= pend && ((((uintptr_t)(key + i)) & 15) == 0)) {
          const uint4 a = *(const uint4*)(key + i), c = *(const uint4*)(key + i + 2);
          kq[u][0] = ((u64)a.y << 32) | a.x; kq[u][1] = ((u64)a.w << 32) | a.z; kq[u][2] = ((u64)c.y << 32) | c.x; kq[u][3] = ((u64)c.w << 32) | c.z;
        } else {
#pragma unroll
          for (int q = 0; q < 4; q++) kq[u][q] = (i + q < pend) ? key[i + q] : 0ULL;
        }
      }
      u32 e[TRC_U][4]; bool look[TRC_U][4]; u64 k48[TRC_U][4];
#pragma unroll
      for (int u = 0; u < TRC_U; u++) {
        const int i = i0 + u * 4096 + (int)threadIdx.x * 4;
#pragma unroll
        for (int q = 0; q < 4; q++) {
          k48[u][q] = trk_k48(kq[u][q], X.bitsR);
          if (L == 2 && chunk == 0) stq[u][q] = (act[u] && i + q < pend) ? ((1u << 16) | (u32)(k48[u][q] >> 40)) : 0xC0000000u;
          look[u][q] = act[u] && (i + q < pend) && (stq[u][q] >> 30) == 0 && ((stq[u][q] >> 16) & 7u) != (u32)L;
          e[u][q] = 0;
          if (look[u][q]) e[u][q] = info[(stq[u][q] & 0xFFFFu) * 256 + (u32)((k48[u][q] >> (40 - 8 * (L - 1))) & 0xFFu)];
        }
      }
#pragma unroll
      for (int u = 0; u < TRC_U; u++) {
        if (!act[u]) continue;
        const int i = i0 + u * 4096 + (int)threadIdx.x * 4;
        bool changed = false;
        u32 runT = 0xFFFFFFFFu, runC = 0;
#pragma unroll
        for (int q = 0; q < 4; q++) {
          u32 tgt = 0xFFFFFFFFu;
          if ((i + q < pend) && (stq[u][q] >> 30) == 0) {
            if (look[u][q]) { stq[u][q] = ((e[u][q] >> 30) == TR_K_EXP) ? ((e[u][q] & 0xFFFFu) | ((u32)L << 16)) : e[u][q]; changed = true; }
            if ((stq[u][q] >> 30) == 0) {
              const int k = (int)(stq[u][q] & 0xFFFFu) - nlo;
              if (k >= 0 && k < TR_NODECHUNK) tgt = (u32)k * 256 + (u32)((k48[u][q] >> (40 - 8 * L)) & 0xFFu);
            }
          }
          if (tgt == runT) runC++;
          else { if (runC && runT != 0xFFFFFFFFu) atomicAdd(&lds[runT], runC); runT = tgt; runC = 1; }
        }
        if (runC && runT != 0xFFFFFFFFu) atomicAdd(&lds[runT], runC);
        if (changed) *(uint4*)(state + i) = make_uint4(stq[u][0], stq[u][1], stq[u][2], stq[u][3]);
      }
    }
    __syncthreads();
    for (int j = threadIdx.x; j < TR_NODECHUNK * 256; j += 1024) {
      const u32 v = lds[j];
      if (v && nlo + (j >> 8) < hi) atomicAdd(&cnt[(int64_t)(nlo + (j >> 8)) * 256 + (j & 255)], v);
    }
    __syncthreads();
  }
}

template <int TILE_, int MAXB_, bool FAST>
__device__ __forceinline__ void trk_scatter_body(const KeySrc& X, const u32* __restrict__ stateAll, u64* __restrict__ elemAll, const BwtArrays& A, const TrieArrays& T, int bitsG) {
  constexpr int ITEMS_ = TILE_ / 1024;
  const int b = bw_row_block(A, blockIdx.y);
  if ((T.meta[(int64_t)b * TR_META + 1] <= TRS_FASTB) != FAST) return;
  const int w0 = A.d_w[b];
  const int W = A.d_m[b] - w0;
  const int tbase = blockIdx.x * TILE_;
  if (tbase >= W) return;
  __shared__ u32 tc2[MAXB_ / 2];
  __shared__ u32 gdelta[MAXB_];
  __shared__ u64 stage[TILE_];
  __shared__ uint16_t stageB[TILE_];
  __shared__ u32 scan[32];
  const int32_t* meta = T.meta + (int64_t)b * TR_META;
  const int nB = meta[1];
  const bool hasState = meta[10 + 2] > meta[2 + 2];
  for (int i = threadIdx.x; i < (nB + 1) / 2; i += 1024) tc2[i] = 0;
  __syncthreads();
  const u64* key = X.key + (int64_t)b * A.NS + w0;
  const u32* val = X.val + (int64_t)b * A.NS + w0;
  const u32* state = stateAll + (int64_t)b * A.NS;
  const u32* info = T.info + (int64_t)b * T.MN * 256;
  u32* rank = A.rank + (int64_t)b * A.NS;
  const u64 lowMask = (1ULL << bitsG) - 1ULL;
  u64 el[ITEMS_]; u32 bp[ITEMS_];
  u64 k48v[ITEMS_]; u32 svv[ITEMS_], stv[ITEMS_];
#pragma unroll
  for (int r = 0; r < ITEMS_; r++) {
    const int i = tbase + r * 1024 + threadIdx.x;
    k48v[r] = 0; svv[r] = 0; stv[r] = 0xC0000000u;
    if (i < W) {
      k48v[r] = trk_k48(key[i], X.bitsR);
      svv[r] = val[i];
      stv[r] = hasState ? state[i] : ((1u << 16) | (u32)(k48v[r] >> 40));
    }
  }
#pragma unroll
  for (int r = 0; r < ITEMS_; r++) {
    const int i = tbase + r * 1024 + threadIdx.x;
    if (i < W && (stv[r] >> 30) == 0) stv[r] = info[(stv[r] & 0xFFFFu) * 256 + (u32)((k48v[r] >> (40 - 8 * (int)((stv[r] >> 16) & 7u))) & 0xFFu)];
  }
#pragma unroll
  for (int r = 0; r < ITEMS_; r++) {
    const int i = tbase + r * 1024 + threadIdx.x;
    bp[r] = 0xFFFFFFFFu;
    el[r] = 0;
    if (i < W) {
      const u64 k48 = k48v[r];
      const u32 sv = svv[r];
      const u32 st = stv[r];
      if ((st >> 30) == TR_K_TERM) {
        if (!(st & TR_UNCHANGED)) rank[sv] = (st & 0xFFFFFFu) | BW_LIVE;
      } else {
        const u32 bk = st & 0xFFFFu;
        const int skip = (int)((st >> 16) & 7u);
        el[r] = (((k48 << 16) << (8 * skip)) & ~lowMask) | (u64)sv;
        const u32 old = atomicAdd(&tc2[bk >> 1], (bk & 1u) ? 65536u : 1u);
        bp[r] = bk | (((bk & 1u) ? (old >> 16) : (old & 0xFFFFu)) << 16);
      }
    }
  }
  __syncthreads();
  {
    const int per = 2 * ((nB + 2047) / 2048);
    const int j0 = threadIdx.x * per;
    u32 mine = 0;
    for (int j = j0; j < j0 + per && j < nB; j += 2) { const u32 w = tc2[j >> 1]; mine += (w & 0xFFFFu) + (w >> 16); }
    u32 total;
    u32 run = kz_wg_excl_sum(mine, scan, &total);
    const u32* bStart = T.bStart + (int64_t)b * T.MB;
    u32* bFill = T.bFill + (int64_t)b * T.MB;
    for (int j = j0; j < j0 + per && j < nB; j += 2) {
      const u32 w = tc2[j >> 1];
      const u32 c0 = w & 0xFFFFu, c1 = w >> 16;
      if (c0) gdelta[j] = bStart[j] + atomicAdd(&bFill[j], c0) - run;
      const u32 r1 = run + c0;
      if (c1) gdelta[j + 1] = bStart[j + 1] + atomicAdd(&bFill[j + 1], c1) - r1;
      tc2[j >> 1] = run | (r1 << 16);
      run = r1 + c1;
    }
    if (threadIdx.x == 0) scan[31] = total;
  }
  __syncthreads();
  const u32 total = scan[31];
#pragma unroll
  for (int r = 0; r < ITEMS_; r++) {
    if (bp[r] != 0xFFFFFFFFu) {
      const u32 bk = bp[r] & 0xFFFFu;
      const u32 w = tc2[bk >> 1];
      const u32 slot = ((bk & 1u) ? (w >> 16) : (w & 0xFFFFu)) + (bp[r] >> 16);
      stage[slot] = el[r]; stageB[slot] = (uint16_t)bk;
    }
  }
  __syncthreads();
  u64* elem = elemAll + (int64_t)b * A.NS;
#pragma unroll
  for (int r = 0; r < ITEMS_; r++) {
    const u32 slot = (u32)r * 1024 + threadIdx.x;
    if (slot < total) elem[gdelta[stageB[slot]] + slot] = stage[slot];
  }
}

__global__ __launch_bounds__(1024) void k_trk_scatter(KeySrc X, const u32* __restrict__ stateAll, u64* __restrict__ elemAll, BwtArrays A, TrieArrays T, int bitsG) { trk_scatter_body<TRS_TILE, TR_MAXB, false>(X, stateAll, elemAll, A, T, bitsG); }
__global__ __launch_bounds__(1024) void k_trk_scatter_f(KeySrc X, const u32* __restrict__ stateAll, u64* __restrict__ elemAll, BwtArrays A, TrieArrays T, int bitsG) { trk_scatter_body<TRS_TILE / 2, TRS_FASTB, true>(X, stateAll, elemAll, A, T, bitsG); }

__global__ void k_bwt_emit(const u8* __restrict__ src, int64_t srcStride, u8* __restrict__ dst, int64_t dstStride,
                           BwtArrays A, int32_t* d_lenOut, int32_t* d_flag, int B) {
  const int lin = blockIdx.y * gridDim.x + blockIdx.x;
  const int sg = lin / (8 * (int)gridDim.x), r8 = lin % (8 * (int)gridDim.x);
  const int b = B < 0 ? (int)blockIdx.y : sg * 8 + (r8 & 7);
  const int chunk = B < 0 ? (int)blockIdx.x : r8 >> 3;
  if (B >= 0 && b >= B) return;
  const int n = A.d_n[b];
  const u8* s = src + (int64_t)b * srcStride;
  u8* d = dst + (int64_t)b * dstStride;
  const int64_t off = (int64_t)b * A.NS;
  if (n < 2) {
    if (chunk == 0 && threadIdx.x == 0) { d_flag[b] = 0; d_lenOut[b] = n; if (n == 1) d[0] = s[0]; }
    return;
  }
  int logBlockSize = kz_ilog2((u32)n);
  if ((n & (n - 1)) != 0) logBlockSize++;
  const int pIndexSize = (logBlockSize + 7) >> 3;
  const int chunks = (n < 256) ? 1 : 8;
  const int hdr = 1 + chunks * pIndexSize;
  const u32* rank = A.rank + off;
  const u32* sa = A.sa + off;
  const int p = (int)rank[0];
  if (chunk == 0 && threadIdx.x == 0) {
    const int logNbChunks = (chunks == 8) ? 3 : 0;
    d[0] = (u8)((logNbChunks << 2) | (pIndexSize - 1));
    const int st = n / chunks;
    const int step = (st * chunks != n) ? st + 1 : st;
    int idx = 1;
    for (int k = 0; k < chunks; k++) {
      const int pi = (int)rank[(int64_t)k * step];
      for (int shift = (pIndexSize - 1) << 3; shift >= 0; shift -= 8) d[idx++] = (u8)(pi >> shift);
    }
    d[hdr] = s[n - 1];
    d_lenOut[b] = hdr + n;
    d_flag[b] = 1;
  }
  for (int j = chunk * blockDim.x + threadIdx.x; j < n; j += gridDim.x * blockDim.x) {
    if (j == p) continue;
    const u32 sv = sa[j];
    const u8 c = s[sv - 1];
    d[hdr + ((j < p) ? j + 1 : j)] = c;
  }
}

#define TR_DMAX_LIMIT 7
#define TR_MIN_N 65536
#define TR_MAX_N ((4 << 20) + 65536)
static inline int tr_max_nodes(int maxN) { return 257 + (TR_DMAX_LIMIT - 2) * (maxN / (int)(TR_CAP + 1) + 1); }
static inline int tr_max_buckets(int maxN) {
  const int med = maxN / (int)(TR_MERGE + 1) + 1, big = maxN / (int)(TR_CAP + 1) + 1;
  return med + 2 * (maxN / (int)TR_CAP) + 2 + tr_max_nodes(maxN) + med + (TR_DMAX_LIMIT - 2) * big + big;
}
static inline bool tr_applies(int maxN) {
  return maxN >= TR_MIN_N && maxN <= TR_MAX_N && tr_max_buckets(maxN) <= TR_MAXB && tr_max_nodes(maxN) <= 65535;
}

size_t kz_bwt_forward_scratch(int B, int maxN) {
  const int64_t NS = (int64_t)kz_align((size_t)maxN, RS_TILE);
  const int T = (int)(NS / RS_TILE);
  size_t per = (size_t)NS * (8 * 2 + 4 * 2 + 4 + 4) + (size_t)(T + 4) * (256 * 4 + 12) + 2 * MSD_BINS * 4 + 64 + 11 * 256;
  if (tr_applies(maxN)) per += (size_t)tr_max_nodes(maxN) * (2 * 1024 + 12) + (size_t)TR_MAXB * 20 + TR_META * 4 + 9 * 256;
  return kz_align(per * (size_t)B + 4096 * 16, 4096) + (1 << 20);
}

static inline int gridFor(int n, int per) { int g = (n + per - 1) / per; return g < 1 ? 1 : g; }

static int bwt_forward_run(kz_ctx* ctx, kz_batch& bt, bool allowTrie, bool* trieOverflow) {
  const int B = bt.B;
  int maxN = 0;
  for (int b = 0; b < B; b++) if (bt.h_len[b] > maxN) maxN = bt.h_len[b];
  const int64_t NS = (int64_t)kz_align((size_t)(maxN > 0 ? maxN : 1), RS_TILE);
  const int T = (int)(NS / RS_TILE);
  BwtArrays A;
  A.NS = NS; A.T = T; A.HS = (int64_t)((NS + RSORT_TILE - 1) / RSORT_TILE) * MSD_BINS;
  for (int i = 0; i < 2; i++) {
    A.key[i] = (u64*)kz_arena_alloc(ctx, (size_t)NS * B * 8);
    A.val[i] = (u32*)kz_arena_alloc(ctx, (size_t)NS * B * 4);
  }
  A.rank = (u32*)kz_arena_alloc(ctx, (size_t)NS * B * 4);
  A.sa = (u32*)kz_arena_alloc(ctx, (size_t)NS * B * 4);
  A.tileHist = (u32*)kz_arena_alloc(ctx, (size_t)A.HS * B * 4);
  A.digitBase = (u32*)kz_arena_alloc(ctx, (size_t)B * MSD_BINS * 4);
  A.bucketCnt = (u32*)kz_arena_alloc(ctx, (size_t)B * MSD_BINS * 4);
  A.d_w = (int32_t*)kz_arena_alloc(ctx, (size_t)B * 4);
  A.d_big = (int32_t*)kz_arena_alloc(ctx, (size_t)B * 4);
  A.tileA = (u32*)kz_arena_alloc(ctx, (size_t)T * B * 4);
  A.tileB = (u32*)kz_arena_alloc(ctx, (size_t)T * B * 4);
  A.tileLive = (u32*)kz_arena_alloc(ctx, (size_t)T * B * 4);
  A.d_m = (int32_t*)kz_arena_alloc(ctx, (size_t)B * 4);
  A.d_m2 = (int32_t*)kz_arena_alloc(ctx, (size_t)B * 4);
  int32_t* d_act = (int32_t*)kz_arena_alloc(ctx, (size_t)B * 4);
  A.act = nullptr;
  if (!d_act || !A.d_m2 || !A.tileB || !A.tileLive || !A.sa || !A.d_big || !A.bucketCnt) { snprintf(ctx->err, sizeof(ctx->err), "bwt_forward: arena overflow"); return -KZ_ERR_DEVICE; }
  bool useTrie = allowTrie && ctx->sw.bwtTrie != 0 && tr_applies(maxN);
  TrieArrays TR;
  memset(&TR, 0, sizeof(TR));
  const size_t markTrie = ctx->arenaTop;
  if (useTrie) {
    TR.MN = tr_max_nodes(maxN); TR.MB = TR_MAXB;
    TR.cnt = (u32*)kz_arena_alloc(ctx, (size_t)B * TR.MN * 1024);
    TR.info = (u32*)kz_arena_alloc(ctx, (size_t)B * TR.MN * 1024);
    TR.nodeStart = (u32*)kz_arena_alloc(ctx, (size_t)B * TR.MN * 4);
    TR.bStart = (u32*)kz_arena_alloc(ctx, (size_t)B * TR.MB * 4);
    TR.bCount = (u32*)kz_arena_alloc(ctx, (size_t)B * TR.MB * 4);
    TR.bFill = (u32*)kz_arena_alloc(ctx, (size_t)B * TR.MB * 4);
    TR.bAux = (u32*)kz_arena_alloc(ctx, (size_t)B * TR.MB * 4);
    TR.bG = (u32*)kz_arena_alloc(ctx, (size_t)B * TR.MB * 4);
    TR.nodePfx = (u32*)kz_arena_alloc(ctx, (size_t)B * TR.MN * 4);
    TR.nodeGS = (u32*)kz_arena_alloc(ctx, (size_t)B * TR.MN * 4);
    TR.meta = (int32_t*)kz_arena_alloc(ctx, (size_t)B * TR_META * 4);
    TR.err = (int32_t*)kz_arena_alloc(ctx, 256);
    if (!TR.cnt || !TR.info || !TR.nodeStart || !TR.bStart || !TR.bCount || !TR.bFill || !TR.bAux || !TR.bG || !TR.nodePfx || !TR.nodeGS || !TR.meta || !TR.err) {
      ctx->arenaTop = markTrie;
      useTrie = false;
    }
  }
  A.d_n = bt.d_len;
  hipStream_t st = ctx->stream;
  const u8* src = bt.buf[bt.cur];
  u8* dst = bt.buf[bt.cur ^ 1];

  int bitsR = 1;
  while ((1LL << bitsR) < 2 * (int64_t)maxN + 2) bitsR++;
  int bitsG = 1;
  while ((1LL << bitsG) < (int64_t)maxN) bitsG++;

  const int K0 = 7;
  u64 *kC = A.key[0], *kF = A.key[1];
  u32 *vC = A.val[0], *vF = A.val[1];
  KZ_LAUNCH(ctx, KID_BWT_INIT, k_bwt_init, dim3((B + 255) / 256), dim3(256), A, B);
  const TextSrc X0 = {src, bt.stride, K0};
  int mMax = maxN;
  int h = 0;
  const bool useBuckets = (BK_BITS + bitsR + bitsG <= 64) && (1 << (bitsG > BK_BITS ? bitsG - BK_BITS : 0)) <= MSD_BINS && ctx->sw.bwtBuckets != 0;
  const int nBuckets = 1 << (bitsG > BK_BITS ? bitsG - BK_BITS : 0);
  const int bucketMin = 4096;
  bool windowed = false;
  const u32 gmax = (u32)BK_GMAX;
  const int tilesN = gridFor(maxN, RS_TILE);
  const int Dmax = (ctx->sw.bwtDmax >= 6 && ctx->sw.bwtDmax <= TR_DMAX_LIMIT) ? ctx->sw.bwtDmax : 6;
  const bool noRetire = ctx->sw.bwtRetire == 0;
  const bool trieWinOff = ctx->sw.bwtTrieWin == 0;
  const bool lazyRank = ctx->sw.bwtLazyRank != 0;
  const bool trace = ctx->sw.bwtTrace != 0;
  const int forceOvfRound = ctx->sw.bwtTestTrieOverflow;
  if (useTrie) KZ_HIP(hipMemsetAsync(TR.err, 0, 4, st));
  int nAct = B;
  int32_t* const h_act = ctx->hpin + B + 16;
  for (int round = 0; round < 64 && mMax > 0; round++) {
    const int nbits = (round == 0) ? 8 * K0 : bitsR + bitsG;
    const int passes = (nbits + 7) / 8;
    const int gshift = (round == 0) ? 64 : bitsR;
    const bool buckets = useBuckets && round > 0 && mMax >= bucketMin;
    int wMax = mMax;
    if (round == 0 && useTrie) {
      KZ_HIP(hipMemsetAsync(TR.bFill, 0, (size_t)B * TR.MB * 4, st));
      KZ_HIP(hipMemsetAsync(TR.meta, 0, (size_t)B * TR_META * 4, st));
      KZ_LAUNCH(ctx, KID_TR_HIST16, k_tr_hist16, dim3(2, B), dim3(1024), src, bt.stride, A, TR);
      KZ_LAUNCH(ctx, KID_TR_ASSIGN, k_tr_assign, dim3(B), dim3(256), A, TR, 1, Dmax, 0);
      const int P = B >= 2048 ? 1 : (B >= 1024 ? 2 : 8);
      for (int L = 2; L < Dmax; L++) {
        KZ_LAUNCH(ctx, KID_TR_COUNT, k_tr_count, dim3(P, B), dim3(1024), src, bt.stride, A.val[0], A, TR, L);
        KZ_LAUNCH(ctx, KID_TR_ASSIGN, k_tr_assign, dim3(B), dim3(256), A, TR, L, Dmax, 0);
      }
      KZ_LAUNCH(ctx, KID_TR_SCATTER, k_tr_scatter_f, dim3(gridFor(maxN, TRS_TILE / 2), B), dim3(1024), src, bt.stride, A.val[0], A.key[0], A, TR, bitsG);
      KZ_LAUNCH(ctx, KID_TR_SCATTER, k_tr_scatter, dim3(gridFor(maxN, TRS_TILE), B), dim3(1024), src, bt.stride, A.val[0], A.key[0], A, TR, bitsG);
      const int G = std::max(16, std::min(1024, 8192 / B));
      KZ_LAUNCH(ctx, KID_TR_SORT, k_tr_sort, dim3(G, B), dim3(1024), A.key[0], A, TR, bitsG, lazyRank ? 1 : 0);
      if (lazyRank) KZ_LAUNCH(ctx, KID_TR_SORT, k_tr_sort, dim3(G, B), dim3(1024), A.key[0], A, TR, bitsG, 2);
      wMax = 0;
    } else
    if (buckets) {
      const int rt = gridFor(mMax, RSORT_TILE);
      const int sh = bitsR + BK_BITS;
      KZ_LAUNCH(ctx, KID_MSD_HIST, k_msd_hist, dim3(rt, nAct), dim3(KZ_WG), kC, A, sh);
      KZ_LAUNCH(ctx, KID_MSD_SCAN, k_msd_scan, dim3(nAct), dim3(MSD_BINS), A);
      KZ_HIP(hipMemcpyAsync(ctx->hpin, A.d_big, (size_t)B * 4, hipMemcpyDeviceToHost, st));
      KZ_LAUNCH(ctx, KID_MSD_SCATTER, k_msd_scatter, dim3(rt, nAct), dim3(RSC_WG), kC, vC, kF, vF, A, sh);
      { u64* tk = kC; kC = kF; kF = tk; u32* tv = vC; vC = vF; vF = tv; }
      KZ_LAUNCH(ctx, KID_BUCKET_COUNT_S, k_bucket_count_s, dim3(nBuckets, nAct), dim3(256), kC, vC, A, bitsR, bitsG, gmax);
      KZ_LAUNCH(ctx, KID_BUCKET_COUNT, k_bucket_count, dim3(nBuckets, nAct), dim3(1024), kC, vC, A, bitsR, bitsG, gmax);
      KZ_LAUNCH(ctx, KID_BUCKET_SORT, k_bucket_sort, dim3(nBuckets, nAct), dim3(1024), kC, vC, A, bitsR, bitsG);
      KZ_HIP(kz_stream_sync(ctx, st));
      wMax = 0;
      for (int r = 0; r < nAct; r++) { const int b = A.act ? h_act[r] : r; if (ctx->hpin[b] > wMax) wMax = ctx->hpin[b]; }
      windowed = true;
      if (trace) {
        long long tot = 0; for (int r = 0; r < nAct; r++) tot += ctx->hpin[A.act ? h_act[r] : r];
        fprintf(stderr, "[bwt] round %d: %lld suffixes in oversized buckets, max per block %d\n", round, tot, wMax);
      }
    } else if (windowed) {
      KZ_HIP(hipMemsetAsync(A.d_w, 0, (size_t)B * 4, st));
      windowed = false;
    }
    const bool trieWindow = useTrie && buckets && wMax > 0 && bitsR <= 24 && bitsG <= 24 && !trieWinOff;
    if (trieWindow) {
      const KeySrc XK = {kC, vC, bitsR};
      KZ_HIP(hipMemsetAsync(TR.bFill, 0, (size_t)B * TR.MB * 4, st));
      KZ_HIP(hipMemsetAsync(TR.meta, 0, (size_t)B * TR_META * 4, st));
      KZ_LAUNCH(ctx, KID_TR_HIST16, k_trk_hist16, dim3(2, nAct), dim3(1024), XK, A, TR);
      KZ_LAUNCH(ctx, KID_TR_ASSIGN, k_tr_assign, dim3(nAct), dim3(256), A, TR, 1, 6, 1);
      const int PW = nAct >= 1024 ? 1 : (nAct >= 256 ? 2 : 4);
      for (int L = 2; L < 6; L++) {
        KZ_LAUNCH(ctx, KID_TR_COUNT, k_trk_count, dim3(PW, nAct), dim3(1024), XK, vF, A, TR, L);
        KZ_LAUNCH(ctx, KID_TR_ASSIGN, k_tr_assign, dim3(nAct), dim3(256), A, TR, L, 6, 1);
      }
      KZ_LAUNCH(ctx, KID_TR_SCATTER, k_trk_scatter_f, dim3(gridFor(wMax, TRS_TILE / 2), nAct), dim3(1024), XK, vF, kF, A, TR, bitsG);
      KZ_LAUNCH(ctx, KID_TR_SCATTER, k_trk_scatter, dim3(gridFor(wMax, TRS_TILE), nAct), dim3(1024), XK, vF, kF, A, TR, bitsG);
      const int G = std::max(16, std::min(1024, 8192 / nAct));
      KZ_LAUNCH(ctx, KID_TR_SORT, k_trk_sort, dim3(G, nAct), dim3(1024), kF, A, TR, bitsG);
    } else
    if (wMax > 0) {
      const int tiles = gridFor(wMax, RS_TILE);
      const int rtiles = gridFor(wMax, RSORT_TILE);
      for (int p = 0; p < passes; p++) {
        if (round == 0 && p == 0) {
          KZ_LAUNCH(ctx, KID_RADIX_HIST, k_radix_hist0, dim3(rtiles, nAct), dim3(KZ_WG), A, X0);
          KZ_LAUNCH(ctx, KID_RADIX_SCAN, k_radix_scan, dim3(nAct), dim3(256), A);
          KZ_LAUNCH(ctx, KID_RADIX_SCATTER, k_radix_scatter0, dim3(rtiles, nAct), dim3(RSC_WG), kF, vF, A, X0);
        } else {
        KZ_LAUNCH(ctx, KID_RADIX_HIST, k_radix_hist, dim3(rtiles, nAct), dim3(KZ_WG), kC, A, p * 8);
        KZ_LAUNCH(ctx, KID_RADIX_SCAN, k_radix_scan, dim3(nAct), dim3(256), A);
        KZ_LAUNCH(ctx, KID_RADIX_SCATTER, k_radix_scatter, dim3(rtiles, nAct), dim3(RSC_WG), kC, vC, kF, vF, A, p * 8);
        }
        u64* tk = kC; kC = kF; kF = tk;
        u32* tv = vC; vC = vF; vF = tv;
      }
      KZ_LAUNCH(ctx, KID_SEG_REDUCE, k_seg_reduce, dim3(tiles, nAct), dim3(KZ_WG), kC, A, gshift);
      KZ_LAUNCH(ctx, KID_SEG_SCAN, k_seg_scan, dim3(nAct), dim3(64), A);
      KZ_LAUNCH(ctx, KID_SEG_APPLY, k_seg_apply, dim3(tiles, nAct), dim3(KZ_WG), kC, vC, A, gshift);
    }
    h = (round == 0) ? (useTrie ? 6 : K0) : h * 2;
    KZ_HIP(hipMemsetAsync(A.d_m2, 0, (size_t)B * 4, st));
    KZ_LAUNCH(ctx, KID_LIVE_EMIT, k_live_emit, dim3(tilesN, nAct), dim3(KZ_WG), kF, vF, A, h, bitsR, round == 0 ? 1 : 0, (round == 0 && useTrie && lazyRank) ? TR.meta : (const int32_t*)nullptr);
    { u64* tk = kC; kC = kF; kF = tk; u32* tv = vC; vC = vF; vF = tv; }
    KZ_HIP(hipMemcpyAsync(ctx->hpin, A.d_m2, (size_t)B * 4, hipMemcpyDeviceToHost, st));
    ctx->hpin[B] = 0;
    if (useTrie) KZ_HIP(hipMemcpyAsync(ctx->hpin + B, TR.err, 4, hipMemcpyDeviceToHost, st));
    KZ_HIP(kz_stream_sync(ctx, st));
    mMax = 0;
    for (int b = 0; b < B; b++) if (ctx->hpin[b] > mMax) mMax = ctx->hpin[b];
    if (useTrie && (ctx->hpin[B] != 0 || round == forceOvfRound)) { *trieOverflow = true; return 0; }
    if (trace) {
      long long tot = 0, totN = 0; for (int b = 0; b < B; b++) { tot += ctx->hpin[b]; totN += bt.h_len[b]; }
      fprintf(stderr, "[bwt] round %d h=%d: live %lld of %lld (%.1f%%), max per block %d\n", round, h, tot, totN, 100.0 * tot / (totN ? totN : 1), mMax);
    }
    int32_t* tm = A.d_m; A.d_m = A.d_m2; A.d_m2 = tm;
    if (mMax > 0 && !noRetire) {
      int cnt = 0;
      for (int b = 0; b < B; b++) if (ctx->hpin[b] > 0) h_act[cnt++] = b;
      if (cnt < B) {
        KZ_HIP(hipMemcpyAsync(d_act, h_act, (size_t)cnt * 4, hipMemcpyHostToDevice, st));
        A.act = d_act;
        nAct = cnt;
      }
    }
  }
  if (mMax > 0) { snprintf(ctx->err, sizeof(ctx->err), "bwt_forward: suffix sort did not converge"); return -KZ_ERR_PROCESS_BLOCK; }
  {
    const int rows8 = (B + 7) / 8 * 8;
    const bool xcd = rows8 <= KZ_MAX_BATCH;
    KZ_LAUNCH(ctx, KID_BWT_EMIT, k_bwt_emit, dim3(gridFor(maxN, 256 * 8), xcd ? rows8 : B), dim3(256), src, bt.stride, dst, bt.stride, A, bt.d_len2, bt.d_flag, xcd ? B : -1);
  }
  KZ_HIP(hipGetLastError());
  bt.cur ^= 1;
  { int32_t* t = bt.d_len; bt.d_len = bt.d_len2; bt.d_len2 = t; }
  return 0;
}

int kz_stage_bwt_forward(kz_ctx* ctx, kz_batch& bt) {
  const size_t mark = ctx->arenaTop;
  bool overflow = false;
  int rc = bwt_forward_run(ctx, bt, true, &overflow);
  if (rc == 0 && overflow) {
    ctx->arenaTop = mark;
    overflow = false;
    rc = bwt_forward_run(ctx, bt, false, &overflow);
  }
  return rc;
}
```

kanzi_amd/csrc/kz_internal.h:

```cpp
#pragma once
#include <hip/hip_runtime.h>
#include <stdint.h>
#include <stdio.h>
#include <string.h>
#include <vector>
#include <condition_variable>
#include <deque>
#include <functional>
#include <map>
#include <set>
#include <mutex>
#include <thread>
#include "../../include/kanzi_hip.h"

enum KzKernelId { KID_ANS_ENC_CHUNK, KID_ANS_ENC_SCAN, KID_ANS_ENC_CONCAT, KID_ANS_DEC_INDEX, KID_ANS_DEC_CHUNK, KID_ANS_DEC_FIN, KID_MASK_LEN, KID_PASSTHROUGH, KID_FRAME_PREPARE, KID_COPY_BYTES, KID_FRAME_DECIDE, KID_FRAME_HEADER, KID_FRAME_PARSE, KID_COPY_PAYLOAD, KID_BWT_INIT, KID_RADIX_HIST, KID_RADIX_SCAN, KID_RADIX_SCATTER, KID_SEG_REDUCE, KID_SEG_SCAN, KID_SEG_APPLY, KID_LIVE_EMIT, KID_BWT_EMIT, KID_BWTI_PARSE, KID_BWTI_HIST, KID_BWTI_SCAN, KID_BWTI_SCATTER, KID_BWTI_WALK1, KID_BWTI_RESOLVE, KID_BWTI_COPY, KID_BWTI_LITERAL, KID_BWTI_FIN, KID_SBRT_LAST2, KID_SBRT_SCAN, KID_SBRT_REPLAY, KID_COPY_LEN, KID_SBRT_INVERSE, KID_ZRLT_F1, KID_ZRLT_F2, KID_ZRLT_F3, KID_ZRLT_FFIN, KID_ZRLT_I1, KID_ZRLT_I2, KID_ZRLT_I3, KID_ZRLT_IFIN, KID_RLT_F0, KID_RLT_FSCAN, KID_RLT_F1, KID_RLT_FSUM, KID_RLT_F3, KID_RLT_FTAIL, KID_RLT_I1, KID_RLT_ISCAN, KID_RLT_I2, KID_RLT_ISUM, KID_RLT_I3, KID_RLT_IFIN, KID_HUF_ENC_CHUNK, KID_HUF_DEC_INDEX, KID_HUF_DEC_CHUNK, KID_HUF_DEC_FIN, KID_FPAQ_ENC, KID_FPAQ_PACK, KID_FPAQ_DEC, KID_SRT_HIST, KID_SRT_PREP, KID_SRT_SCATTER, KID_SRT_INV, KID_LZ_FWD, KID_LZ_INV, KID_XXHASH, KID_BLOCK_MAGIC, KID_MM_ANALYZE, KID_MM_EMIT, KID_MM_CHECK, KID_MM_INV, KID_ALIAS_ANALYZE, KID_ALIAS_HIST1, KID_ALIAS_SELECT, KID_ALIAS_EMIT, KID_ALIAS_INV, KID_SKIP_DECIDE, KID_MSD_HIST, KID_MSD_SCAN, KID_MSD_SCATTER, KID_BUCKET_SORT, KID_BUCKET_COUNT, KID_BUCKET_COUNT_S, KID_TR_HIST16, KID_TR_ASSIGN, KID_TR_COUNT, KID_TR_SCATTER, KID_TR_SORT, KID_TEXT_INV, KID_UTF_INV, KID_TEXT_FWD, KID_TEXT_WALK, KID_UTF_FWD, KID_ANS1_HIST, KID_ANS1_NORM, KID_ANS1_HDR, KID_ANS1_ENC, KID_ANS1_DEC_INDEX, KID_ANS1_DEC_TABLE, KID_ANS1_DEC_CHUNK, KID_ANS1_DEC_FIN, KID_RANGE_ENC_CHUNK, KID_RANGE_ENC_FIN, KID_RANGE_DEC, KID_LZP_FWD, KID_LZP_INV, KID_EXE_SETUP, KID_EXE_MAP, KID_EXE_SCAN, KID_EXE_HIST, KID_EXE_DECIDE, KID_EXE_SIZE, KID_EXE_VERDICT, KID_EXE_EMIT, KID_COUNT };
#define KZ_KERNEL_NAMES { "k_ans_enc_chunk", "k_ans_enc_scan", "k_ans_enc_concat", "k_ans_dec_index", "k_ans_dec_chunk", "k_ans_dec_fin", "k_mask_len", "k_passthrough", "k_frame_prepare", "k_copy_bytes", "k_frame_decide", "k_frame_header", "k_frame_parse", "k_copy_payload", "k_bwt_init", "k_radix_hist", "k_radix_scan", "k_radix_scatter", "k_seg_reduce", "k_seg_scan", "k_seg_apply", "k_live_emit", "k_bwt_emit", "k_bwti_parse", "k_bwti_hist", "k_bwti_scan", "k_bwti_scatter", "k_bwti_walk1", "k_bwti_resolve", "k_bwti_copy", "k_bwti_literal", "k_bwti_fin", "k_sbrt_last2", "k_sbrt_scan", "k_sbrt_replay", "k_copy_len", "k_sbrt_inverse", "k_zrlt_f1", "k_zrlt_f2", "k_zrlt_f3", "k_zrlt_ffin", "k_zrlt_i1", "k_zrlt_i2", "k_zrlt_i3", "k_zrlt_ifin", "k_rlt_f0", "k_rlt_fscan", "k_rlt_f1", "k_rlt_fsum", "k_rlt_f3", "k_rlt_ftail", "k_rlt_i1", "k_rlt_iscan", "k_rlt_i2", "k_rlt_isum", "k_rlt_i3", "k_rlt_ifin", "k_huf_enc_chunk", "k_huf_dec_index", "k_huf_dec_chunk", "k_huf_dec_fin", "k_fpaq_enc", "k_fpaq_pack", "k_fpaq_dec", "k_srt_hist", "k_srt_prep", "k_srt_scatter", "k_srt_inv", "k_lz_fwd", "k_lz_inv", "k_xxhash", "k_block_magic", "k_mm_analyze", "k_mm_emit", "k_mm_check", "k_mm_inv", "k_alias_analyze", "k_alias_hist1", "k_alias_select", "k_alias_emit", "k_alias_inv", "k_skip_decide", "k_msd_hist", "k_msd_scan", "k_msd_scatter", "k_bucket_sort", "k_bucket_count", "k_bucket_count_s", "k_tr_hist16", "k_tr_assign", "k_tr_count", "k_tr_scatter", "k_tr_sort", "k_text_inv", "k_utf_inv", "k_text_fwd", "k_text_walk", "k_utf_fwd", "k_ans1_hist", "k_ans1_norm", "k_ans1_hdr", "k_ans1_enc", "k_ans1_dec_index", "k_ans1_dec_table", "k_ans1_dec_chunk", "k_ans1_dec_fin", "k_range_enc_chunk", "k_range_enc_fin", "k_range_dec", "k_lzp_fwd", "k_lzp_inv", "k_exe_setup", "k_exe_map", "k_exe_scan", "k_exe_hist", "k_exe_decide", "k_exe_size", "k_exe_verdict", "k_exe_emit" }
struct kz_switches {
  int blockingWaits = -1;
  int textGpu = -1;
  int textGpuMin = 512;
  int textFwdGpu = -1;
  int textFwdGpuMin = 256;
  int utfGpu = 1;
  int utfFwdGpu = -1;
  int textGpuTrace = 0;
  int fuseMinBlocks = 32;
  int overlapClasses = 3;
  int wideQueues = -1;
  int noSFirst = 0;
  int traceSched = 0;
  int tracePipe = 0;
  int hostChunk = 0;
  int hostChunkDec = 512;
  int hostInvStaged = -1;
  int streamChunk = 0;
  int streamSerial = 0;
  int bwtTrie = -1, bwtTrieWin = -1, bwtBuckets = -1, bwtDmax = -1, bwtRetire = -1;
  int bwtLazyRank = -1;
  int bwtTrace = 0;
  int bwtTestTrieOverflow = -1;
  int fpaqForce = 0;
  int sbrtForm = -1;
};
void kz_switches_read(kz_switches& s);

struct KzPending { hipEvent_t e0, e1; int id; };
struct kz_ctx {
  int device = 0;
  kz_switches sw;
  hipStream_t stream = nullptr;
  hipStream_t side[5] = {nullptr, nullptr, nullptr, nullptr, nullptr};
  hipEvent_t evJoin[5] = {nullptr, nullptr, nullptr, nullptr, nullptr};
  int wideQueues = -1;
  int wideNow = 0;
  uint8_t* arena = nullptr;
  size_t arenaCap = 0, arenaTop = 0;
  int32_t* hpin = nullptr;
  size_t hpinInts = 0;
  char err[512] = {0};
  float stageMs[KZ_MAX_STAGES] = {0};
  int64_t stageAlgBytes[KZ_MAX_STAGES] = {0};
  int nStages = 0;
  int checksum = 0;
  int skipBlocks = 0;
  int dataType = 0;
  int blockSize = 4 * 1024 * 1024;
  bool blockSizeSet = false;
  int entropy = KZ_E_NONE;
  int rltBlockSize = 0;
  int numCUs = 256;
  long long* d_endBits = nullptr;
  bool timing = false;
  bool ktiming = false;
  std::vector<KzPending> pending;
  std::vector<hipEvent_t> evPool;
  double kMs[KID_COUNT] = {0};
  double kMaxMs[KID_COUNT] = {0};
  long long kLaunches[KID_COUNT] = {0};
  std::thread worker;
  std::mutex qmu;
  std::condition_variable qcv;
  std::deque<std::pair<int64_t, std::function<int32_t()>>> queue;
  std::map<int64_t, int32_t> finished;
  std::set<int64_t> collected;
  int64_t collectedBelow = 1;
  int64_t nextJob = 1;
  bool stopWorker = false;
  struct Stage { uint8_t* p = nullptr; size_t cap = 0; };
  Stage pinIn[2], pinOut[2];
  Stage devIn[2], devOut[2];
  Stage hsIn[2], hsOut[2];
  Stage tfIn, tfOut[2];
  hipStream_t tfCopy = nullptr;
  hipStream_t copyUp = nullptr, copyDown = nullptr;
  Stage hiAux[2];
  hipStream_t hiStream[2] = {nullptr, nullptr};
  int blockingWaits = 0;
  hipEvent_t evBlock = nullptr;
};

struct kz_arena_guard { kz_ctx* c; size_t mark; ~kz_arena_guard() { c->arenaTop = mark; } };

#define KZ_HIP(x) do { hipError_t e_ = (x); if (e_ != hipSuccess) { \
  snprintf(ctx->err, sizeof(ctx->err), "%s:%d %s -> %s", __FILE__, __LINE__, #x, hipGetErrorString(e_)); \
  return -KZ_ERR_DEVICE; } } while (0)

static inline hipError_t kz_stream_sync(kz_ctx* ctx, hipStream_t st) {
  if (!ctx->blockingWaits) return hipStreamSynchronize(st);
  if (!ctx->evBlock) { hipError_t e = hipEventCreateWithFlags(&ctx->evBlock, hipEventBlockingSync | hipEventDisableTiming); if (e != hipSuccess) return e; }
  hipError_t e = hipEventRecord(ctx->evBlock, st);
  if (e != hipSuccess) return e;
  return hipEventSynchronize(ctx->evBlock);
}

#define KZ_MAX_PACKED_BLOCK ((1 << 24) - 257)
#define KZ_MAX_BLOCK ((1 << 30) + 1057)
#define KZ_MAX_BATCH 65535
int kz_hpin_reserve(kz_ctx* ctx, size_t ints);
static inline size_t kz_align(size_t v, size_t a) { return (v + a - 1) / a * a; }

int kz_arena_reserve(kz_ctx* ctx, size_t total);
void* kz_arena_alloc(kz_ctx* ctx, size_t bytes);

struct kz_batch {
  int B = 0;
  int maxN = 0;
  int64_t stride = 0;
  uint8_t* buf[2] = {nullptr, nullptr};
  int cur = 0;
  int32_t* d_len = nullptr;
  int32_t* d_len2 = nullptr;
  int32_t* d_flag = nullptr;
  int32_t* d_dtype = nullptr;
  const int32_t* d_rltEnd = nullptr;
  int rltEndAll = 0;
  std::vector<int32_t> h_len;
  int slotRot = 0;
  int prio = 0;
  std::vector<int32_t> h_cost;
};

struct KzPlacement { int wpg = 1; int R = 1; std::vector<int> G, off; const int32_t* d_order = nullptr; };
int kz_place_blocks(kz_ctx*, const kz_batch&, KzPlacement&);

int kz_stage_bwt_forward(kz_ctx*, kz_batch&);
int kz_stage_bwt_inverse(kz_ctx*, kz_batch&);
int kz_stage_sbrt_forward(kz_ctx*, kz_batch&, int mode);
int kz_stage_sbrt_inverse(kz_ctx*, kz_batch&, int mode);
int kz_sbrt_ranks(kz_ctx*, const uint8_t* src, uint8_t* dst, int64_t stride, const int32_t* d_len, int B, int maxN, int mode);
int kz_stage_srt_forward(kz_ctx*, kz_batch&);
int kz_stage_srt_inverse(kz_ctx*, kz_batch&);
int kz_stage_lz_forward(kz_ctx*, kz_batch&, int extra);
int kz_stage_mm_forward(kz_ctx*, kz_batch&);
int kz_stage_mm_inverse(kz_ctx*, kz_batch&, int dstCap);
size_t kz_mm_scratch(int B, int maxN);
int kz_stage_alias_forward(kz_ctx*, kz_batch&, int onlyDNA);
int kz_stage_alias_inverse(kz_ctx*, kz_batch&, int dstCap);
size_t kz_alias_scratch(int B, int maxN, bool decode);
int kz_block_data_types(kz_ctx*, kz_batch&, int init, bool sniff);
int kz_skip_block_flags(kz_ctx*, kz_batch&, int32_t* d_skip);
int kz_stage_lz_inverse(kz_ctx*, kz_batch&, int extra, int dstCap);
int kz_stage_fpaq_encode(kz_ctx*, kz_batch&, uint8_t* out, int64_t outStride, const int32_t* d_hdrBytes, int64_t* d_bits);
int kz_stage_fpaq_decode(kz_ctx*, kz_batch&, const uint8_t* in, int64_t inStride, const int64_t* d_bitOff, const int64_t* d_bitEnd);
int kz_block_hashes(kz_ctx*, const uint8_t* data, int64_t stride, const int32_t* d_len, int B, int kind, unsigned long long* d_hash);
size_t kz_srt_scratch(int B, int maxN);
size_t kz_fpaq_scratch(int B, int maxN);
size_t kz_lz_scratch(int B, int maxN);
int kz_stage_zrlt_forward(kz_ctx*, kz_batch&);
int kz_stage_zrlt_inverse(kz_ctx*, kz_batch&, int dstCap);
int kz_stage_rlt_forward(kz_ctx*, kz_batch&, int entropy);
int kz_stage_rlt_inverse(kz_ctx*, kz_batch&, int dstCap);
size_t kz_rlt_scratch(int B, int maxN);
int kz_stage_lzp_forward(kz_ctx*, kz_batch&);
int kz_stage_lzp_inverse(kz_ctx*, kz_batch&, int dstCap);
size_t kz_lzp_scratch(int B, int maxN);
int kz_stage_exe_forward(kz_ctx*, kz_batch&);
int kz_stage_exe_inverse(kz_ctx*, kz_batch&, int dstCap);
size_t kz_exe_scratch(int B, int maxN, bool decode);
int kz_stage_ans0_encode(kz_ctx*, kz_batch&, uint8_t* out, int64_t outStride, const int32_t* d_hdrBytes, int64_t* d_bits);
int kz_stage_ans0_decode(kz_ctx*, kz_batch&, const uint8_t* in, int64_t inStride, const int64_t* d_bitOff, const int64_t* d_bitEnd);
int kz_stage_ans1_encode(kz_ctx*, kz_batch&, uint8_t* out, int64_t outStride, const int32_t* d_hdrBytes, int64_t* d_bits);
int kz_stage_ans1_decode(kz_ctx*, kz_batch&, const uint8_t* in, int64_t inStride, const int64_t* d_bitOff, const int64_t* d_bitEnd);
size_t kz_ans1_scratch(int B, int maxN, bool decode);
int64_t kz_ans1_max_stream_bytes(int n);
int kz_stage_range_encode(kz_ctx*, kz_batch&, uint8_t* out, int64_t outStride, const int32_t* d_hdrBytes, int64_t* d_bits);
int kz_stage_range_decode(kz_ctx*, kz_batch&, const uint8_t* in, int64_t inStride, const int64_t* d_bitOff, const int64_t* d_bitEnd);
size_t kz_range_scratch(int B, int maxN, bool decode);
int64_t kz_range_max_stream_bytes(int n);
int kz_stage_huffman_encode(kz_ctx*, kz_batch&, uint8_t* out, int64_t outStride, const int32_t* d_hdrBytes, int64_t* d_bits);
int kz_stage_huffman_decode(kz_ctx*, kz_batch&, const uint8_t* in, int64_t inStride, const int64_t* d_bitOff, const int64_t* d_bitEnd);

size_t kz_bwt_forward_scratch(int B, int maxN);
size_t kz_bwt_inverse_scratch(int B, int maxN);
size_t kz_sbrt_scratch(int B, int maxN);
size_t kz_zrlt_scratch(int B, int maxN);
size_t kz_ans_scratch(int B, int maxN);

hipEvent_t kz_ev(kz_ctx* ctx);
void kz_ktimer_flush(kz_ctx* ctx);
#define KZ_LAUNCH(ctx, kid, kernel, grid, block, ...) do { \
  hipEvent_t a_ = nullptr, b_ = nullptr; \
  if ((ctx)->ktiming) { a_ = kz_ev(ctx); b_ = kz_ev(ctx); (void)hipEventRecord(a_, (ctx)->stream); } \
  hipLaunchKernelGGL(kernel, grid, block, 0, (ctx)->stream, __VA_ARGS__); \
  if ((ctx)->ktiming) { (void)hipEventRecord(b_, (ctx)->stream); (ctx)->pending.push_back({a_, b_, kid}); } } while (0)

bool kz_is_host_transform(int type);
int kz_host_block_data_type(const uint8_t* p, int n, int init);
int kz_host_transform_forward(int type, int entropyType, int blockSize, int* dataType, const uint8_t* src, int n, uint8_t* dst, int dstCap, int* produced);
int kz_host_transform_inverse(int type, int blockSize, const uint8_t* src, int n, uint8_t* dst, int dstCap, int* produced);
size_t kz_text_gpu_scratch_per_block(int blockSize);
size_t kz_text_fwd_gpu_scratch(int B, int blockSize, int maxLen);
int kz_utf_fwd_gpu(kz_ctx* ctx, kz_batch& bt, const std::vector<int32_t>& take, std::vector<int32_t>& done);
bool kz_text_fwd_gpu_applies(kz_ctx* ctx, uint64_t transformType, uint32_t entropyType, int nBlocks);
struct TextFwdJob;
TextFwdJob* kz_text_fwd_gpu_new();
void kz_text_fwd_gpu_free(TextFwdJob*);
int kz_text_fwd_gpu_classify(kz_ctx* ctx, kz_batch& bt, int blockSize, const std::vector<int32_t>& take, std::vector<int32_t>& keeps,
                             std::vector<int32_t>& declined, TextFwdJob& J);
int kz_text_fwd_gpu_launch(kz_ctx* ctx, kz_batch& bt, TextFwdJob& J);
int kz_text_fwd_gpu_finish(kz_ctx* ctx, kz_batch& bt, TextFwdJob& J, std::vector<int32_t>& done);
size_t kz_utf_gpu_scratch_per_block(int maxLen);
int kz_stage_utf_inverse_gpu(kz_ctx* ctx, kz_batch& bt, int dstCap, const std::vector<int32_t>& take, std::vector<int32_t>& done);
int kz_stage_text_inverse_gpu(kz_ctx* ctx, kz_batch& bt, int blockSize, int dstCap, bool variant1, const std::vector<int32_t>& take, std::vector<int32_t>& done, int form);
void kz_parallel_for(int n, int maxThreads, void (*fn)(int, void*), void* arg);
int kz_usable_cpus();
struct HostPre;
int kz_stage_reserve(kz_ctx* ctx, kz_ctx::Stage& s, size_t need, bool pinned);
int32_t kz_encode_blocks_pre(kz_ctx* ctx, uint64_t transformType, uint32_t entropyType, int32_t blockSize, const uint8_t* in, int64_t inStride,
                             const int32_t* lengths, int32_t nBlocks, uint8_t* out, int64_t outStride, kz_block_result* results, int32_t memKind, const HostPre* pre);
HostPre* kz_host_prestage(kz_ctx* ctx, uint64_t transformType, uint32_t entropyType, int32_t blockSize, const uint8_t* hsrc, int64_t hstride,
                          const int32_t* lengths, int32_t nBlocks, int slotId);
void kz_host_pre_free(HostPre* p);

void kz_stage_begin(kz_ctx*, hipEvent_t* e0);
void kz_stage_end(kz_ctx*, hipEvent_t e0, int stageId, int64_t algBytes);
```

Before: 4797 MB/s.

## Add wide unstable first pass and flat interpolation sort to BWT bucket sorts

Pulls the LDS radix sort in the bucket and trie sort kernels into a shared helper. By default it starts with a 13-bit unstable pass that uses packed LDS atomics before the 9-bit stable passes. For trie buckets whose keys are spread evenly, it also adds a flat path: an interpolation scatter into 8192 slots, chosen after a sum-of-squares flatness test. The goal is fewer LDS radix passes per bucket, paid for with atomics, extra reductions and more code complexity. Both paths are on by default through KZ_BWT_LDSFIN, and trace counters are added as well.

```diff
diff --git a/kanzi_amd/csrc/kz_api.hip b/kanzi_amd/csrc/kz_api.hip
--- a/kanzi_amd/csrc/kz_api.hip
+++ b/kanzi_amd/csrc/kz_api.hip
@@ -59,6 +59,7 @@
   s.streamSerial = flag("KZ_STREAM_SERIAL");
   s.bwtTrie = num("KZ_BWT_TRIE", -1); s.bwtTrieWin = num("KZ_BWT_TRIEWIN", -1); s.bwtBuckets = num("KZ_BWT_BUCKETS", -1);
   s.bwtDmax = num("KZ_BWT_DMAX", -1); s.bwtRetire = num("KZ_BWT_RETIRE", -1); s.bwtLazyRank = num("KZ_BWT_LAZYRANK", -1);
+  s.bwtLdsFin = num("KZ_BWT_LDSFIN", -1);
   s.bwtTrace = flag("KZ_BWT_TRACE");
   s.bwtTestTrieOverflow = digit("KZ_BWT_TEST_TRIE_OVERFLOW", 0, 9, -1);
   { const char* f = getenv("KZ_FPAQ_FORCE"); s.fpaqForce = f ? ((f[0] == 'w' || f[0] == 'W' || f[0] == '1') ? 1 : ((f[0] == 'l' || f[0] == 'L' || f[0] == '2') ? 2 : 0)) : 0; }
diff --git a/kanzi_amd/csrc/kz_bwt_fwd.hip b/kanzi_amd/csrc/kz_bwt_fwd.hip
--- a/kanzi_amd/csrc/kz_bwt_fwd.hip
+++ b/kanzi_amd/csrc/kz_bwt_fwd.hip
@@ -444,8 +444,150 @@
 #define BK_SORT 0x40000000u
 static_assert(RSC_WG == MSD_BINS, "k_msd_scatter geometry");
 
+#define BK_WBITS 13
+#define BK_LDS_WAVES 16
+static_assert((1 << BK_WBITS) * 2 == BK_LDS_WAVES * BK_DBINS * 2, "the wide table fills cw exactly");
+template <int ROWS>
+__device__ __forceinline__ int bw_lds_sort(u64 (&k)[ROWS], const int R, const int cnt, const int lo, const int nbits, const bool wide,
+                                           u64* __restrict__ buf, uint16_t* __restrict__ cw, u32* __restrict__ wsum, u32* __restrict__ wscan,
+                                           int* __restrict__ skip) {
+  constexpr int WG = BK_LDS_WAVES * 64;
+  const int wave = threadIdx.x >> 6, lane = kz_lane();
+  const int base = wave * R * 64;
+  const uint64_t lt = kz_lanemask_lt();
+  u32* const cw32 = (u32*)cw;
+  u32 dr[ROWS];
+  int done = 0, sp = 0;
+  if (wide && nbits > 0) {
+    const int w = min(BK_WBITS, nbits);
+    const u32 dmask = (1u << w) - 1u;
+    for (int i = threadIdx.x; i < BK_LDS_WAVES * BK_DBINS / 2; i += WG) cw32[i] = 0;
+    __syncthreads();
+#pragma unroll
+    for (int r = 0; r < ROWS; r++) {
+      if (r < R) {
+        const int idx = base + r * 64 + lane;
+        const bool valid = idx < cnt;
+        const u32 dg = (u32)(k[r] >> lo) & dmask;
+        const uint64_t vm = kz_ballot(valid);
+        if (vm == 0) continue;
+        const u32 d0 = (u32)__builtin_amdgcn_readfirstlane((int)dg);
+        const bool uni = kz_ballot(valid && dg == d0) == vm;
+        const u32 hsh = (dg & 1u) * 16u;
+        u32 old = 0;
+        if (uni ? lane == 0 : valid) old = atomicAdd(&cw32[dg >> 1], (uni ? (u32)__popcll(vm) : 1u) << hsh);
+        if (uni) old = (u32)__builtin_amdgcn_readfirstlane((int)old);
+        const u32 pos = ((old >> hsh) & 0xFFFFu) + (uni ? (u32)__popcll(vm & lt) : 0u);
+        dr[r] = dg | (pos << 16);
+      }
+    }
+    __syncthreads();
+    constexpr int WPT = (1 << BK_WBITS) / 2 / WG;
+    u32 wv[WPT]; u32 mine = 0; bool one = false;
+#pragma unroll
+    for (int q = 0; q < WPT; q++) {
+      wv[q] = cw32[threadIdx.x * WPT + q];
+      const u32 c0 = wv[q] & 0xFFFFu, c1 = wv[q] >> 16;
+      mine += c0 + c1;
+      one = one || c0 == (u32)cnt || c1 == (u32)cnt;
+    }
+    if (one) skip[0] = 1;
+    const u32 inc = kz_wave_incl_sum(mine);
+    if (lane == 63) wscan[wave] = inc;
+    __syncthreads();
+    if (!skip[0]) {
+      u32 run = inc - mine;
+      for (int wv_ = 0; wv_ < wave; wv_++) run += wscan[wv_];
+#pragma unroll
+      for (int q = 0; q < WPT; q++) {
+        const u32 c0 = wv[q] & 0xFFFFu, c1 = wv[q] >> 16;
+        cw32[threadIdx.x * WPT + q] = run | ((run + c0) << 16);
+        run += c0 + c1;
+      }
+      __syncthreads();
+#pragma unroll
+      for (int r = 0; r < ROWS; r++) {
+        if (r < R) {
+          const int idx = base + r * 64 + lane;
+          if (idx < cnt) buf[cw[dr[r] & 0xFFFF] + (dr[r] >> 16)] = k[r];
+        }
+      }
+      __syncthreads();
+#pragma unroll
+      for (int r = 0; r < ROWS; r++) {
+        if (r < R) {
+          const int idx = base + r * 64 + lane;
+          if (idx < cnt) k[r] = buf[idx];
+        }
+      }
+      __syncthreads();
+    }
+    done = w; sp = 1;
+  }
+  const int passes = (nbits - done + BK_DBITS - 1) / BK_DBITS;
+  for (int p = 0; p < passes; p++) {
+    const int shift = lo + done + BK_DBITS * p;
+    for (int i = threadIdx.x; i < BK_LDS_WAVES * BK_DBINS / 2; i += WG) cw32[i] = 0;
+    __syncthreads();
+#pragma unroll
+    for (int r = 0; r < ROWS; r++) {
+      if (r < R) {
+        const int idx = base + r * 64 + lane;
+        const bool valid = idx < cnt;
+        const u32 dg = (u32)(k[r] >> shift) & (BK_DBINS - 1);
+        const uint64_t vm = kz_ballot(valid);
+        if (vm == 0) continue;
+        const u32 d0 = (u32)__builtin_amdgcn_readfirstlane((int)dg);
+        const bool uni = kz_ballot(valid && dg == d0) == vm;
+        const uint64_t peers = uni ? (valid ? vm : 0ULL) : bw_match<BK_DBITS>(dg, valid);
+        u32 pre = 0;
+        if (valid) pre = cw[wave * BK_DBINS + dg];
+        const u32 rnk = pre + (u32)__popcll(peers & lt);
+        if (valid && (peers >> lane) == 1ULL) cw[wave * BK_DBINS + dg] = (uint16_t)(pre + (u32)__popcll(peers));
+        dr[r] = dg | (rnk << 16);
+      }
+    }
+    __syncthreads();
+    static_assert(BK_DBINS <= WG, "one digit per thread");
+    u32 mine = 0;
+    if (threadIdx.x < BK_DBINS) {
+#pragma unroll
+      for (int w = 0; w < BK_LDS_WAVES; w++) mine += cw[w * BK_DBINS + threadIdx.x];
+      if (mine == (u32)cnt) skip[sp + p] = 1;
+    }
+    const u32 inc = kz_wave_incl_sum(mine);
+    if (lane == 63 && wave < BK_DBINS / 64) wsum[wave] = inc;
+    __syncthreads();
+    if (skip[sp + p]) continue;
+    if (threadIdx.x < BK_DBINS) {
+      u32 run = inc - mine;
+      for (int w = 0; w < wave; w++) run += wsum[w];
+#pragma unroll
+      for (int w = 0; w < BK_LDS_WAVES; w++) { const u32 cv = cw[w * BK_DBINS + threadIdx.x]; cw[w * BK_DBINS + threadIdx.x] = (uint16_t)run; run += cv; }
+    }
+    __syncthreads();
+#pragma unroll
+    for (int r = 0; r < ROWS; r++) {
+      if (r < R) {
+        const int idx = base + r * 64 + lane;
+        if (idx < cnt) buf[cw[wave * BK_DBINS + (dr[r] & 0xFFFF)] + (dr[r] >> 16)] = k[r];
+      }
+    }
+    __syncthreads();
+#pragma unroll
+    for (int r = 0; r < ROWS; r++) {
+      if (r < R) {
+        const int idx = base + r * 64 + lane;
+        if (idx < cnt) k[r] = buf[idx];
+      }
+    }
+    __syncthreads();
+  }
+  return passes;
+}
+
 template <int WAVES, int ROWS>
-__device__ __forceinline__ void bucket_body(const u64* __restrict__ keyS, const u32* __restrict__ valS, const BwtArrays& A, int bitsR, int bitsG) {
+__device__ __forceinline__ void bucket_body(const u64* __restrict__ keyS, const u32* __restrict__ valS, const BwtArrays& A, int bitsR, int bitsG, int fin) {
   const int b = bw_row_block(A, blockIdx.y);
   const u32 d = blockIdx.x;
   const u32 bc0 = A.bucketCnt[b * MSD_BINS + d];
@@ -465,7 +607,7 @@
   const int base = wave * R * 64;
   const uint64_t lt = kz_lanemask_lt();
   const u64 kbase = (u64)d << (bitsR + BK_BITS);
-  u64 k[ROWS]; u32 dr[ROWS];
+  u64 k[ROWS];
 #pragma unroll
   for (int r = 0; r < ROWS; r++) {
     const int idx = base + r * 64 + lane;
@@ -473,79 +615,9 @@
     if (r < R && idx < cnt) k[r] = ((keyS[off + bo + idx] - kbase) << bitsG) | (u64)valS[off + bo + idx];
   }
   {
+    static_assert(WAVES == BK_LDS_WAVES, "bw_lds_sort geometry");
     if (threadIdx.x < 8) skip[threadIdx.x] = 0;
-    const int keyBits = bitsR + BK_BITS;
-    const int passes = (keyBits + BK_DBITS - 1) / BK_DBITS;
-    for (int p = 0; p < passes; p++) {
-      const int shift = bitsG + BK_DBITS * p;
-      for (int i = threadIdx.x; i < WAVES * BK_DBINS / 2; i += WAVES * 64) ((u32*)&cw[0][0])[i] = 0;
-      __syncthreads();
-#pragma unroll
-      for (int r = 0; r < ROWS; r++) {
-        if (r < R) {
-          const int idx = base + r * 64 + lane;
-          const bool valid = idx < cnt;
-          const u32 dg = (u32)(k[r] >> shift) & (BK_DBINS - 1);
-          const uint64_t vm = kz_ballot(valid);
-          if (vm == 0) continue;
-          const u32 d0 = (u32)__builtin_amdgcn_readfirstlane((int)dg);
-          const bool uni = kz_ballot(valid && dg == d0) == vm;
-          const uint64_t peers = uni ? (valid ? vm : 0ULL) : bw_match<BK_DBITS>(dg, valid);
-          u32 pre = 0;
-          if (valid) pre = cw[wave][dg];
-          const u32 rnk = pre + (u32)__popcll(peers & lt);
-          if (valid && (peers >> lane) == 1ULL) cw[wave][dg] = (uint16_t)(pre + (u32)__popcll(peers));
-          dr[r] = dg | (rnk << 16);
-        }
-      }
-      __syncthreads();
-      constexpr int DPT = (BK_DBINS + WAVES * 64 - 1) / (WAVES * 64);
-      u32 c[DPT][WAVES]; u32 tot[DPT]; u32 mine = 0;
-#pragma unroll
-      for (int q = 0; q < DPT; q++) {
-        const int dg = threadIdx.x * DPT + q;
-        tot[q] = 0;
-        if (dg < BK_DBINS) {
-#pragma unroll
-          for (int w = 0; w < WAVES; w++) { c[q][w] = cw[w][dg]; tot[q] += c[q][w]; }
-          if (tot[q] == (u32)cnt) skip[p] = 1;
-        }
-        mine += tot[q];
-      }
-      const u32 inc = kz_wave_incl_sum(mine);
-      if (lane == 63 && wave < BK_DBINS / 64) wsum[wave] = inc;
-      __syncthreads();
-      if (skip[p]) continue;
-      {
-        u32 run = inc - mine;
-        for (int w = 0; w < wave && w < BK_DBINS / 64; w++) run += wsum[w];
-#pragma unroll
-        for (int q = 0; q < DPT; q++) {
-          const int dg = threadIdx.x * DPT + q;
-          if (dg < BK_DBINS) {
-#pragma unroll
-            for (int w = 0; w < WAVES; w++) { cw[w][dg] = (uint16_t)run; run += c[q][w]; }
-          }
-        }
-      }
-      __syncthreads();
-#pragma unroll
-      for (int r = 0; r < ROWS; r++) {
-        if (r < R) {
-          const int idx = base + r * 64 + lane;
-          if (idx < cnt) buf[cw[wave][dr[r] & 0xFFFF] + (dr[r] >> 16)] = k[r];
-        }
-      }
-      __syncthreads();
-#pragma unroll
-      for (int r = 0; r < ROWS; r++) {
-        if (r < R) {
-          const int idx = base + r * 64 + lane;
-          if (idx < cnt) k[r] = buf[idx];
-        }
-      }
-      __syncthreads();
-    }
+    bw_lds_sort<ROWS>(k, R, cnt, bitsG, bitsR + BK_BITS, (fin & 1) != 0, buf, &cw[0][0], wsum, wH, skip);
 #pragma unroll
     for (int r = 0; r < ROWS; r++) {
       if (r < R) {
@@ -607,8 +679,8 @@
     }
   }
 }
-__global__ __launch_bounds__(1024, 8) void k_bucket_sort(const u64* __restrict__ keyS, const u32* __restrict__ valS, BwtArrays A, int bitsR, int bitsG) {
-  bucket_body<16, BK_CAP / 1024>(keyS, valS, A, bitsR, bitsG);
+__global__ __launch_bounds__(1024, 8) void k_bucket_sort(const u64* __restrict__ keyS, const u32* __restrict__ valS, BwtArrays A, int bitsR, int bitsG, int fin) {
+  bucket_body<16, BK_CAP / 1024>(keyS, valS, A, bitsR, bitsG, fin);
 }
 
 #define BK_GMAX 256
@@ -1158,8 +1230,27 @@
 __device__ __forceinline__ bool tr_lazy_candidate(const int32_t* meta) { return meta[0] == 256 && meta[18] == 0; }
 #define TRQ_WAVES 16
 #define TRQ_ROWS 8
+#define TRF_WIDE 1
+#define TRF_FLAT 2
+#define TRF_TRACE 4
+#define TRF_SBITS 13
+#define TRF_SLOTS (1 << TRF_SBITS)
+#ifndef TRF_W
+#define TRF_W 8
+#endif
+#define TR_META_PATHS 24
+static_assert(TR_META_PATHS + 5 <= TR_META, "spare words of the trie round's counters");
+__device__ __forceinline__ void tr_store0(u32* __restrict__ rank, u32* __restrict__ sa, u32 bo, u32 sv, u32 hh, u32 slot, bool live, bool lazy, u32 pstep, u32& liveMine) {
+  if (!lazy) rank[sv] = (bo + hh) | (live ? BW_LIVE : 0u);
+  else {
+    const u32 q = sv / pstep;
+    if (q * pstep == sv && q < 8u) rank[sv] = (bo + hh) | (live ? BW_LIVE : 0u);
+    liveMine += live ? 1u : 0u;
+  }
+  if (!live) sa[bo + slot] = sv;
+}
 template <bool KEYS>
-__device__ __forceinline__ void tr_sort_body(const u64* __restrict__ elemAll, const BwtArrays& A, const TrieArrays& T, int bitsG, int lazyMode) {
+__device__ __forceinline__ void tr_sort_body(const u64* __restrict__ elemAll, const BwtArrays& A, const TrieArrays& T, int bitsG, int lazyMode, int fin) {
   const int b = bw_row_block(A, blockIdx.y);
   const int nB = T.meta[(int64_t)b * TR_META + 1];
   const bool lazyCand = !KEYS && lazyMode != 0 && tr_lazy_candidate(T.meta + (int64_t)b * TR_META);
@@ -1173,7 +1264,12 @@
   __shared__ u32 wsum[BK_DBINS / 64];
   __shared__ u32 wH[TRQ_WAVES], wS[TRQ_WAVES];
   __shared__ u64 redO[TRQ_WAVES], redA[TRQ_WAVES];
+  __shared__ u64 redMin[KEYS ? 1 : TRQ_WAVES], redMax[KEYS ? 1 : TRQ_WAVES];
   __shared__ int skip[8];
+  static_assert(TRQ_WAVES == BK_LDS_WAVES, "bw_lds_sort geometry");
+  const bool wide = (fin & TRF_WIDE) != 0;
+  const bool flatCand = !KEYS && (fin & TRF_FLAT) != 0 && tr_lazy_candidate(T.meta + (int64_t)b * TR_META);
+  u32 nFlat = 0, nCheap = 0, nBoth = 0, nFall = 0, nStable = 0;
   const int wave = threadIdx.x >> 6, lane = kz_lane();
   const int64_t off = (int64_t)b * A.NS;
   const u64* elem = elemAll + off;
@@ -1192,86 +1288,119 @@
     const int rows = (cnt + 63) >> 6;
     const int R = (rows + TRQ_WAVES - 1) / TRQ_WAVES;
     const int base = wave * R * 64;
-    u64 k[TRQ_ROWS]; u32 dr[TRQ_ROWS];
-    u64 vo = 0, va = ~0ULL;
+    u64 k[TRQ_ROWS];
+    u64 vo = 0, va = ~0ULL, kmin = ~0ULL, kmax = 0;
 #pragma unroll
     for (int r = 0; r < TRQ_ROWS; r++) {
       const int idx = base + r * 64 + lane;
       k[r] = ~0ULL;
-      if (r < R && idx < cnt) { k[r] = elem[bo + idx]; vo |= k[r]; va &= k[r]; }
+      if (r < R && idx < cnt) {
+        k[r] = elem[bo + idx]; vo |= k[r]; va &= k[r];
+        if (flatCand) { const u64 kv = k[r] >> bitsG; kmin = kv < kmin ? kv : kmin; kmax = kv > kmax ? kv : kmax; }
+      }
     }
     for (int dd = 32; dd > 0; dd >>= 1) { vo |= __shfl_xor(vo, dd, 64); va &= __shfl_xor(va, dd, 64); }
+    if (flatCand) {
+      for (int dd = 32; dd > 0; dd >>= 1) {
+        const u64 on = __shfl_xor(kmin, dd, 64), ox = __shfl_xor(kmax, dd, 64);
+        kmin = on < kmin ? on : kmin; kmax = ox > kmax ? ox : kmax;
+      }
+    }
     if (threadIdx.x < 8) skip[threadIdx.x] = 0;
-    if (lane == 0) { redO[wave] = vo; redA[wave] = va; }
+    if (lane == 0) { redO[wave] = vo; redA[wave] = va; if (flatCand) { redMin[KEYS ? 0 : wave] = kmin; redMax[KEYS ? 0 : wave] = kmax; } }
     __syncthreads();
     vo = 0; va = ~0ULL;
 #pragma unroll
     for (int w = 0; w < TRQ_WAVES; w++) { vo |= redO[w]; va &= redA[w]; }
     const u64 diff = (vo ^ va) >> bitsG;
-    int passes = 0, lowBit = 0;
+    bool finished = false;
+    if (!KEYS && flatCand && diff) {
+      kmin = ~0ULL; kmax = 0;
+#pragma unroll
+      for (int w = 0; w < TRQ_WAVES; w++) { const u64 on = redMin[KEYS ? 0 : w], ox = redMax[KEYS ? 0 : w]; kmin = on < kmin ? on : kmin; kmax = ox > kmax ? ox : kmax; }
+      const u64 range = kmax - kmin + 1;
+      const int L = (int)__builtin_clzll(range);
+      const u32 M = (u32)(0x1p62 / ((double)(u32)((range << L) >> 32) + 1.0)) - 1u;
+      static_assert(TRF_SBITS == 13, "the shift below");
+      u32* const cw32 = (u32*)&cw[0][0];
+      uint16_t* const st16 = &cw[0][0];
+      for (int i = threadIdx.x; i < TRF_SLOTS / 2; i += TRQ_WAVES * 64) cw32[i] = 0;
+      __syncthreads();
+      const auto slotOf = [&](u64 e) { return min(__umulhi((u32)((((e >> bitsG) - kmin) << L) >> 32), M) >> 17, (u32)TRF_SLOTS - 1u); };
+#pragma unroll
+      for (int r = 0; r < TRQ_ROWS; r++) {
+        const int idx = base + r * 64 + lane;
+        if (r < R && idx < cnt) { const u32 slot = slotOf(k[r]); atomicAdd(&cw32[slot >> 1], 1u << ((slot & 1u) * 16u)); }
+      }
+      __syncthreads();
+      constexpr int WPT = TRF_SLOTS / 2 / (TRQ_WAVES * 64);
+      u32 wv[WPT]; u32 mine = 0, sq = 0;
+#pragma unroll
+      for (int q = 0; q < WPT; q++) {
+        wv[q] = cw32[threadIdx.x * WPT + q];
+        const u32 c0 = wv[q] & 0xFFFFu, c1 = wv[q] >> 16;
+        mine += c0 + c1; sq += c0 * c0 + c1 * c1;
+      }
+      const u32 inc = kz_wave_incl_sum(mine);
+      sq = kz_wave_sum(sq);
+      if (lane == 63) { wH[wave] = inc; wS[wave] = sq; }
+      __syncthreads();
+      u32 sqAll = 0;
+#pragma unroll
+      for (int w = 0; w < TRQ_WAVES; w++) sqAll += wS[w];
+      const bool flat = __builtin_amdgcn_readfirstlane((int)(sqAll <= (u32)TRF_W * (u32)cnt)) != 0;
+      if (flat) {
+        u32 run = inc - mine;
+        for (int w = 0; w < wave; w++) run += wH[w];
+#pragma unroll
+        for (int q = 0; q < WPT; q++) {
+          const u32 c0 = wv[q] & 0xFFFFu, c1 = wv[q] >> 16;
+          cw32[threadIdx.x * WPT + q] = run | ((run + c0) << 16);
+          run += c0 + c1;
+        }
+        __syncthreads();
+#pragma unroll
+        for (int r = 0; r < TRQ_ROWS; r++) {
+          const int idx = base + r * 64 + lane;
+          if (r < R && idx < cnt) {
+            const u32 slot = slotOf(k[r]);
+            const u32 hsh = (slot & 1u) * 16u;
+            buf[(atomicAdd(&cw32[slot >> 1], 1u << hsh) >> hsh) & 0xFFFFu] = k[r];
+          }
+        }
+        __syncthreads();
+#pragma unroll
+        for (int r = 0; r < TRQ_ROWS; r++) {
+          const int idx = base + r * 64 + lane;
+          if (r < R && idx < cnt) {
+            const u32 slot = slotOf(k[r]);
+            const u64 kv = k[r] >> bitsG;
+            const int gs = slot ? (int)st16[slot - 1] : 0;
+            const int ge = (int)st16[slot];
+            u32 rk = 0, eq = 0;
+            int j = gs;
+            for (; j + 4 <= ge; j += 4) {
+              const u64 e0 = buf[j] >> bitsG, e1 = buf[j + 1] >> bitsG, e2 = buf[j + 2] >> bitsG, e3 = buf[j + 3] >> bitsG;
+              rk += (e0 < kv) + (e1 < kv) + (e2 < kv) + (e3 < kv);
+              eq += (e0 == kv) + (e1 == kv) + (e2 == kv) + (e3 == kv);
+            }
+            for (; j < ge; j++) { const u64 ej = buf[j] >> bitsG; rk += (ej < kv) ? 1u : 0u; eq += (ej == kv) ? 1u : 0u; }
+            const u32 hh = (u32)gs + rk;
+            tr_store0(rank, sa, bo, (u32)(k[r] & vmask), hh, hh, eq > 1, lazy, pstep, liveMine);
+          }
+        }
+        finished = true;
+        nFlat++;
+      } else nFall++;
+    }
+    if (!finished) {
+    int nbits = 0, lowBit = 0;
     if (diff) {
       lowBit = (int)__builtin_ctzll(diff);
-      const int hiBit = 63 - (int)__builtin_clzll(diff);
-      passes = (hiBit - lowBit + BK_DBITS) / BK_DBITS;
-    }
-    for (int p = 0; p < passes; p++) {
-      const int shift = bitsG + lowBit + BK_DBITS * p;
-      for (int i = threadIdx.x; i < TRQ_WAVES * BK_DBINS / 2; i += TRQ_WAVES * 64) ((u32*)&cw[0][0])[i] = 0;
-      __syncthreads();
-#pragma unroll
-      for (int r = 0; r < TRQ_ROWS; r++) {
-        if (r < R) {
-          const int idx = base + r * 64 + lane;
-          const bool valid = idx < cnt;
-          const u32 dg = (u32)(k[r] >> shift) & (BK_DBINS - 1);
-          const uint64_t vm = kz_ballot(valid);
-          if (vm == 0) continue;
-          const u32 d0 = (u32)__builtin_amdgcn_readfirstlane((int)dg);
-          const bool uni = kz_ballot(valid && dg == d0) == vm;
-          const uint64_t peers = uni ? (valid ? vm : 0ULL) : bw_match<BK_DBITS>(dg, valid);
-          u32 pre = 0;
-          if (valid) pre = cw[wave][dg];
-          const u32 rnk = pre + (u32)__popcll(peers & lt);
-          if (valid && (peers >> lane) == 1ULL) cw[wave][dg] = (uint16_t)(pre + (u32)__popcll(peers));
-          dr[r] = dg | (rnk << 16);
-        }
-      }
-      __syncthreads();
-      static_assert(BK_DBINS <= TRQ_WAVES * 64, "one digit per thread");
-      u32 mine = 0;
-      if (threadIdx.x < BK_DBINS) {
-#pragma unroll
-        for (int w = 0; w < TRQ_WAVES; w++) mine += cw[w][threadIdx.x];
-        if (mine == (u32)cnt) skip[p] = 1;
-      }
-      const u32 inc = kz_wave_incl_sum(mine);
-      if (lane == 63 && wave < BK_DBINS / 64) wsum[wave] = inc;
-      __syncthreads();
-      if (skip[p]) continue;
-      if (threadIdx.x < BK_DBINS) {
-        u32 run = inc - mine;
-        for (int w = 0; w < wave; w++) run += wsum[w];
-#pragma unroll
-        for (int w = 0; w < TRQ_WAVES; w++) { const u32 cv = cw[w][threadIdx.x]; cw[w][threadIdx.x] = (uint16_t)run; run += cv; }
-      }
-      __syncthreads();
-#pragma unroll
-      for (int r = 0; r < TRQ_ROWS; r++) {
-        if (r < R) {
-          const int idx = base + r * 64 + lane;
-          if (idx < cnt) buf[cw[wave][dr[r] & 0xFFFF] + (dr[r] >> 16)] = k[r];
-        }
-      }
-      __syncthreads();
-#pragma unroll
-      for (int r = 0; r < TRQ_ROWS; r++) {
-        if (r < R) {
-          const int idx = base + r * 64 + lane;
-          if (idx < cnt) k[r] = buf[idx];
-        }
-      }
-      __syncthreads();
-    }
+      nbits = 64 - (int)__builtin_clzll(diff) - lowBit;
+    }
+    const int stable = bw_lds_sort<TRQ_ROWS>(k, R, cnt, bitsG + lowBit, nbits, wide, buf, &cw[0][0], wsum, wH, skip);
+    if (!(flatCand && diff)) { if (!wide) nStable++; else if (stable) nBoth++; else nCheap++; }
 #pragma unroll
     for (int r = 0; r < TRQ_ROWS; r++) {
       if (r < R) {
@@ -1325,15 +1454,8 @@
           const bool headN = (idx + 1 >= cnt) || ((nextk >> bitsG) != (k[r] >> bitsG));
           const bool live = !(hh == (u32)idx && headN);
           const u32 sv = (u32)(k[r] & vmask);
-          if (!KEYS) {
-            if (!lazy) rank[sv] = (bo + hh) | (live ? BW_LIVE : 0u);
-            else {
-              const u32 q = sv / pstep;
-              if (q * pstep == sv && q < 8u) rank[sv] = (bo + hh) | (live ? BW_LIVE : 0u);
-              liveMine += live ? 1u : 0u;
-            }
-            if (!live) sa[bo + (u32)idx] = sv;
-          } else {
+          if (!KEYS) tr_store0(rank, sa, bo, sv, hh, (u32)idx, live, lazy, pstep, liveMine);
+          else {
             u32 g, headSlot, slot;
             if (segs) {
               g = (aux << (8 * (3 - skipB))) | (u32)(k[r] >> gsh);
@@ -1347,7 +1469,16 @@
         if (sbr) carS = (u32)(rowBase + 63 - (int)__builtin_clzll(sbr)) + 1;
       }
     }
-    __syncthreads();
+    }
+    __syncthreads();
+  }
+  if (!KEYS && (fin & TRF_TRACE) != 0 && lazyMode != 2 && threadIdx.x == 0) {
+    int32_t* tc = T.meta + TR_META_PATHS;
+    if (nFlat) atomicAdd(&tc[0], (int32_t)nFlat);
+    if (nCheap) atomicAdd(&tc[1], (int32_t)nCheap);
+    if (nBoth) atomicAdd(&tc[2], (int32_t)nBoth);
+    if (nFall) atomicAdd(&tc[3], (int32_t)nFall);
+    if (nStable) atomicAdd(&tc[4], (int32_t)nStable);
   }
   if (!KEYS && lazy) {
     if (kz_ballot(liveMine != 0) != 0) {
@@ -1356,8 +1487,8 @@
     }
   }
 }
-__global__ __launch_bounds__(1024, 8) void k_tr_sort(const u64* __restrict__ elemAll, BwtArrays A, TrieArrays T, int bitsG, int lazyMode) { tr_sort_body<false>(elemAll, A, T, bitsG, lazyMode); }
-__global__ __launch_bounds__(1024, 8) void k_trk_sort(const u64* __restrict__ elemAll, BwtArrays A, TrieArrays T, int bitsG) { tr_sort_body<true>(elemAll, A, T, bitsG, 0); }
+__global__ __launch_bounds__(1024, 8) void k_tr_sort(const u64* __restrict__ elemAll, BwtArrays A, TrieArrays T, int bitsG, int lazyMode, int fin) { tr_sort_body<false>(elemAll, A, T, bitsG, lazyMode, fin); }
+__global__ __launch_bounds__(1024, 8) void k_trk_sort(const u64* __restrict__ elemAll, BwtArrays A, TrieArrays T, int bitsG, int fin) { tr_sort_body<true>(elemAll, A, T, bitsG, 0, fin); }
 
 struct KeySrc { const u64* key; const u32* val; int bitsR; };
 __device__ __forceinline__ u64 trk_k48(u64 key, int bitsR) { return ((key >> bitsR) << 24) | (key & ((1ULL << bitsR) - 1ULL)); }
@@ -1730,6 +1861,7 @@
   const bool trieWinOff = ctx->sw.bwtTrieWin == 0;
   const bool lazyRank = ctx->sw.bwtLazyRank != 0;
   const bool trace = ctx->sw.bwtTrace != 0;
+  const int fin = ((ctx->sw.bwtLdsFin < 0 ? 3 : ctx->sw.bwtLdsFin) & (TRF_WIDE | TRF_FLAT)) | (trace ? TRF_TRACE : 0);
   const int forceOvfRound = ctx->sw.bwtTestTrieOverflow;
   if (useTrie) KZ_HIP(hipMemsetAsync(TR.err, 0, 4, st));
   int nAct = B;
@@ -1753,8 +1885,9 @@
       KZ_LAUNCH(ctx, KID_TR_SCATTER, k_tr_scatter_f, dim3(gridFor(maxN, TRS_TILE / 2), B), dim3(1024), src, bt.stride, A.val[0], A.key[0], A, TR, bitsG);
       KZ_LAUNCH(ctx, KID_TR_SCATTER, k_tr_scatter, dim3(gridFor(maxN, TRS_TILE), B), dim3(1024), src, bt.stride, A.val[0], A.key[0], A, TR, bitsG);
       const int G = std::max(16, std::min(1024, 8192 / B));
-      KZ_LAUNCH(ctx, KID_TR_SORT, k_tr_sort, dim3(G, B), dim3(1024), A.key[0], A, TR, bitsG, lazyRank ? 1 : 0);
-      if (lazyRank) KZ_LAUNCH(ctx, KID_TR_SORT, k_tr_sort, dim3(G, B), dim3(1024), A.key[0], A, TR, bitsG, 2);
+      KZ_LAUNCH(ctx, KID_TR_SORT, k_tr_sort, dim3(G, B), dim3(1024), A.key[0], A, TR, bitsG, lazyRank ? 1 : 0, fin);
+      if (lazyRank) KZ_LAUNCH(ctx, KID_TR_SORT, k_tr_sort, dim3(G, B), dim3(1024), A.key[0], A, TR, bitsG, 2, fin);
+      if (trace) KZ_HIP(hipMemcpyAsync(ctx->hpin + B + 1, TR.meta + TR_META_PATHS, 5 * 4, hipMemcpyDeviceToHost, st));
       wMax = 0;
     } else
     if (buckets) {
@@ -1767,7 +1900,7 @@
       { u64* tk = kC; kC = kF; kF = tk; u32* tv = vC; vC = vF; vF = tv; }
       KZ_LAUNCH(ctx, KID_BUCKET_COUNT_S, k_bucket_count_s, dim3(nBuckets, nAct), dim3(256), kC, vC, A, bitsR, bitsG, gmax);
       KZ_LAUNCH(ctx, KID_BUCKET_COUNT, k_bucket_count, dim3(nBuckets, nAct), dim3(1024), kC, vC, A, bitsR, bitsG, gmax);
-      KZ_LAUNCH(ctx, KID_BUCKET_SORT, k_bucket_sort, dim3(nBuckets, nAct), dim3(1024), kC, vC, A, bitsR, bitsG);
+      KZ_LAUNCH(ctx, KID_BUCKET_SORT, k_bucket_sort, dim3(nBuckets, nAct), dim3(1024), kC, vC, A, bitsR, bitsG, fin);
       KZ_HIP(kz_stream_sync(ctx, st));
       wMax = 0;
       for (int r = 0; r < nAct; r++) { const int b = A.act ? h_act[r] : r; if (ctx->hpin[b] > wMax) wMax = ctx->hpin[b]; }
@@ -1795,7 +1928,7 @@
       KZ_LAUNCH(ctx, KID_TR_SCATTER, k_trk_scatter_f, dim3(gridFor(wMax, TRS_TILE / 2), nAct), dim3(1024), XK, vF, kF, A, TR, bitsG);
       KZ_LAUNCH(ctx, KID_TR_SCATTER, k_trk_scatter, dim3(gridFor(wMax, TRS_TILE), nAct), dim3(1024), XK, vF, kF, A, TR, bitsG);
       const int G = std::max(16, std::min(1024, 8192 / nAct));
-      KZ_LAUNCH(ctx, KID_TR_SORT, k_trk_sort, dim3(G, nAct), dim3(1024), kF, A, TR, bitsG);
+      KZ_LAUNCH(ctx, KID_TR_SORT, k_trk_sort, dim3(G, nAct), dim3(1024), kF, A, TR, bitsG, fin);
     } else
     if (wMax > 0) {
       const int tiles = gridFor(wMax, RS_TILE);
@@ -1831,6 +1964,10 @@
     if (trace) {
       long long tot = 0, totN = 0; for (int b = 0; b < B; b++) { tot += ctx->hpin[b]; totN += bt.h_len[b]; }
       fprintf(stderr, "[bwt] round %d h=%d: live %lld of %lld (%.1f%%), max per block %d\n", round, h, tot, totN, 100.0 * tot / (totN ? totN : 1), mMax);
+      if (round == 0 && useTrie) {
+        const int32_t* pc = ctx->hpin + B + 1;
+        fprintf(stderr, "[bwt] round 0 buckets: flat %d, cheap pass only %d, cheap + stable %d, fallback after flatness test %d, stable only %d\n", pc[0], pc[1], pc[2], pc[3], pc[4]);
+      }
     }
     int32_t* tm = A.d_m; A.d_m = A.d_m2; A.d_m2 = tm;
     if (mMax > 0 && !noRetire) {
diff --git a/kanzi_amd/csrc/kz_internal.h b/kanzi_amd/csrc/kz_internal.h
--- a/kanzi_amd/csrc/kz_internal.h
+++ b/kanzi_amd/csrc/kz_internal.h
@@ -37,6 +37,7 @@
   int streamSerial = 0;
   int bwtTrie = -1, bwtTrieWin = -1, bwtBuckets = -1, bwtDmax = -1, bwtRetire = -1;
   int bwtLazyRank = -1;
+  int bwtLdsFin = -1;
   int bwtTrace = 0;
   int bwtTestTrieOverflow = -1;
   int fpaqForce = 0;
```

Result: no change. 4802 MB/s (median of 2 runs) (+0.1%).
